# LiWentomng/OrientedRepPoints

Measured on AMD Instinct MI355X. Metric: images/sec (1024x1024 DOTA, R-50 FPN), higher is better.
Workload: dtype f32; 1 GPU; configs[1]: OrientedRepPoints R-50 FPN inference, 1024x1024 patch, 15 classes, bs=1/GPU, nms_pre=2000, score_thr=0.05, rnms iou_thr=0.4, max_per_img=2000; random-init weights, head biases calibrated to ~2000 dets/img; global_batch=1, parallelism=replicas x1 (image-parallel, no collective), images_in_flight_per_gpu=4

## Files before the change

include/orp_hip.h:

```cpp
#ifndef ORP_HIP_H_
#define ORP_HIP_H_

#include <stddef.h>
#include <stdint.h>

#ifdef __cplusplus
extern "C" {
#endif

#define ORP_OK 0
#define ORP_EINVAL (-1)
#define ORP_EWORKSPACE (-2)
#define ORP_ETOOBIG (-3)

const char* orp_version(void);

#define ORP_NMS_MAX_BOXES 131072
size_t orp_rnms_workspace_bytes(int n);
int orp_rnms(const float* dets, int n, float iou_thr, int flavor, int presorted, int order_out,
             int64_t* keep_out, int32_t* num_keep, void* workspace, size_t workspace_bytes, void* stream);

size_t orp_rnms_batched_workspace_bytes(int n_total, int nseg, int max_seg);
int orp_rnms_batched(const float* dets, int n_total, const int32_t* seg_offsets, int nseg, int max_seg,
                     float iou_thr, int flavor, int64_t* keep_out, int32_t* num_keep,
// ... 94 lines not shown
int orp_dcn_backward_multi(const orp_dcn_bwd_level* levels_host, int nlevels, int batch, int c_in, int c_out,
                           const float* weight, float* grad_weight, int need_input_grads, int kh, int kw, int stride_h,
                           int stride_w, int pad_h, int pad_w, int dil_h, int dil_w, void* workspace,
                           size_t workspace_bytes, void* stream);
int orp_dcn_backward_multi_ex(const orp_dcn_bwd_level* levels_host, const float* const* masks_host,
                              float* const* grad_masks_host, int io_dtype, int nlevels, int batch, int c_in, int c_out,
                              const float* weight, float* grad_weight, int need_input_grads, int kh, int kw, int stride_h,
                              int stride_w, int pad_h, int pad_w, int dil_h, int dil_w, void* workspace,
                              size_t workspace_bytes, void* stream);

int orp_dcn_im2col(const float* input, const float* offset, const float* mask, int batch, int c_in, int height,
                   int width, int kh, int kw, int stride_h, int stride_w, int pad_h, int pad_w, int dil_h, int dil_w,
                   int deformable_groups, float* columns, void* stream);
int orp_dcn_col2im(const float* grad_columns, const float* input, const float* offset, const float* mask, int batch,
                   int c_in, int height, int width, int kh, int kw, int stride_h, int stride_w, int pad_h, int pad_w,
                   int dil_h, int dil_w, int deformable_groups, float* grad_input, float* grad_offset, float* grad_mask,
                   void* stream);
int orp_dcn_im2col_f64(const double* input, const double* offset, const double* mask, int batch, int c_in, int height,
                       int width, int kh, int kw, int stride_h, int stride_w, int pad_h, int pad_w, int dil_h, int dil_w,
                       int deformable_groups, double* columns, void* stream);
int orp_dcn_col2im_f64(const double* grad_columns, const double* input, const double* offset, const double* mask, int batch,
                       int c_in, int height, int width, int kh, int kw, int stride_h, int stride_w, int pad_h, int pad_w,
                       int dil_h, int dil_w, int deformable_groups, double* grad_input, double* grad_offset, double* grad_mask,
                       void* stream);
int orp_dcn_col2im_nhwc(const float* grad_columns_t, const float* input_nhwc, const float* offset, int batch, int c_in,
                        int height, int width, int kh, int kw, int stride_h, int stride_w, int pad_h, int pad_w,
                        int dil_h, int dil_w, float* grad_input_nhwc, float* grad_offset, void* stream);

size_t orp_point_assign_workspace_bytes(int n);
int orp_point_assign(const float* points, int n, const float* gts, int k, float scale, int pos_num, int64_t* gt_inds,
                     void* workspace, size_t workspace_bytes, void* stream);
size_t orp_max_iou_assign_workspace_bytes(int k);
int orp_max_iou_assign(const float* overlaps_nk, int n, int k, float pos_iou_thr, float neg_iou_lo, float neg_iou_hi,
                       float min_pos_iou, int gt_max_assign_all, int64_t* gt_inds, float* max_overlaps,
                       void* workspace, size_t workspace_bytes, void* stream);
int orp_apaa_feature_dissimilarity(const float* const* feats_host, const int* heights_host, const int* widths_host,
                                   const float* strides_host, int num_levels, int channels, const float* pts18,
                                   const int32_t* img_index, const int32_t* level_index, int p, float* out,
                                   void* stream);
int orp_apaa_select(const float* quality, const int64_t* pos_gt_inds, const int32_t* pos_level, int p, int num_gt,
                    int num_level, int per_level_topk, double top_ratio, uint8_t* keep, void* stream);

typedef struct { const float* data; float* grad; int height; int width; float stride; } orp_level_desc;
int orp_pointset_target(const int64_t* gt_inds, const uint8_t* valid, int batch, int n, const float* gt_boxes,
                        const int64_t* gt_labels, const int32_t* gt_offset, const float* proposals, int dim,
                        float pos_weight, int64_t* labels, float* label_weights, float* rbbox_gt, float* pos_proposals,
                        float* proposal_weights, int64_t* gt_inds_out, int32_t* counts, void* stream);
int orp_points_from_offsets(const orp_level_desc* levels_host, int nlevels, int batch, int channels, int mode, float* out,
                            void* stream);
int orp_gather_levels(const orp_level_desc* levels_host, int nlevels, int batch, int channels, const int64_t* index, int p,
                      int mode, float* out, void* stream);
int orp_gather_levels_backward(const orp_level_desc* levels_host, int nlevels, int batch, int channels, const int64_t* index,
                               int p, int mode, const float* grad_out, void* stream);
int orp_outline_samples(const float* corners, int p, int n, const float* ratios, float* out, void* stream);

int orp_border_rows(const float* pts18, const float* gt8, const float* weight, int p, float* row_sum, float* row_cnt,
                    float* gdir, void* stream);
int orp_giou_rows(const float* gious, const float* grad18, const float* weight, const int64_t* seg, const float* denom, int p,
                  float loss_weight, float* contrib, float* gsave, void* stream);
int orp_segment_finish(const float* row_val, const float* row_cnt, const int64_t* seg, int p, int nseg, const float* denom,
                       float loss_weight, int mode, float* loss, float* scale, void* stream);

size_t orp_poly_nms_f64_workspace_bytes(int n);
int orp_poly_nms_f64(const double* dets_sorted, int n, double iou_thr, int64_t* keep_out, int32_t* num_keep,
                     void* workspace, size_t workspace_bytes, void* stream);

size_t orp_poly_nms_f64_batched_workspace_bytes(int n_total, int nseg, int max_seg);
int orp_poly_nms_f64_batched(const double* dets, int n_total, const int32_t* seg_offsets, int nseg, int max_seg,
                             double iou_thr, int hbb_prefilter, int presorted, int64_t* keep_out, int32_t* num_keep,
                             void* workspace, size_t workspace_bytes, void* stream);

int orp_scene_tiles(const uint8_t* scene, int height, int width, long long row_stride_bytes, const int32_t* origins,
                    int num_tiles, int tile, const float* mean_host, const float* std_host, int to_rgb, int out_dtype,
                    void* out, void* stream);
int orp_scene_tiles_resized(const uint8_t* scene, int height, int width, long long row_stride_bytes, const int32_t* origins,
                            int num_tiles, int src_w, int src_h, int new_w, int new_h, int pad_w, int pad_h, const int32_t* x_i0,
                            const float* x_w1, const int32_t* y_i0, const float* y_w1, const float* mean_host,
                            const float* std_host, int to_rgb, int out_dtype, void* out, void* stream);
int orp_scene_tiles_flip(const uint8_t* scene, int height, int width, long long row_stride_bytes, const int32_t* origins,
                         int num_tiles, int tile, const float* mean_host, const float* std_host, int to_rgb, int out_dtype,
                         void* out, void* stream);
int orp_scene_tiles_resized_flip(const uint8_t* scene, int height, int width, long long row_stride_bytes, const int32_t* origins,
                                 int num_tiles, int src_w, int src_h, int new_w, int new_h, int pad_w, int pad_h,
                                 const int32_t* x_i0, const float* x_w1, const int32_t* y_i0, const float* y_w1,
                                 const float* mean_host, const float* std_host, int to_rgb, int out_dtype, void* out,
                                 void* stream);
size_t orp_scene_collect_workspace_bytes(int num_tiles, int num_classes);
int orp_scene_collect(const float* packed, int num_tiles, int max_rows, const int32_t* origins, double rate, int num_classes,
                      int capacity_rows, double* dets, int32_t* seg_offsets, int32_t* src, int32_t* flag, void* workspace,
                      size_t workspace_bytes, void* stream);

int orp_voc_best_match_f64(const double* dets, const int32_t* det_image, int num_dets, const double* gts,
                           const int32_t* gt_offsets, int num_images, double* ovmax, int32_t* jmax, void* stream);

int orp_soft_rnms_host(const float* dets_host, int m, float iou_thr, int method, float sigma, float min_score,
                       float* out_host, int* num_out);

typedef struct { const float* input; float* output; int height; int width; } orp_norm_level;
size_t orp_groupnorm_workspace_bytes(const orp_norm_level* levels_host, int nlevels, int batch, int channels, int groups);
int orp_groupnorm_act_multi(const orp_norm_level* levels_host, int nlevels, int batch, int channels, int groups,
                            const float* gamma, const float* beta, float eps, int relu, void* workspace,
                            size_t workspace_bytes, void* stream);
int orp_groupnorm_act_multi_ex(const orp_norm_level* levels, const float* const* gammas_host,
                               const float* const* betas_host, int nlevels, int batch, int channels, int groups,
                               float eps, int relu, void* workspace, size_t workspace_bytes, void* stream);
int orp_groupnorm_act_multi_nhwc(const orp_norm_level* levels, const float* const* gammas_host,
                                 const float* const* betas_host, float* const* nhwc_out_host, int nlevels, int batch,
                                 int channels, int groups, float eps, int relu, void* workspace, size_t workspace_bytes,
                                 void* stream);
size_t orp_groupnorm_cl_workspace_bytes(const orp_norm_level* levels_host, int nlevels, int batch, int channels, int groups);
int orp_groupnorm_act_multi_cl(const orp_norm_level* levels, const float* const* gammas_host, const float* const* betas_host,
                               int nlevels, int batch, int channels, int groups, float eps, int relu, void* workspace,
                               size_t workspace_bytes, void* stream);
int orp_groupnorm_act_multi_cl_amax(const orp_norm_level* levels, const float* const* gammas_host, const float* const* betas_host,
                                    int nlevels, int batch, int channels, int groups, float eps, int relu, const int* slots_host,
                                    uint32_t* amax_out, int nslots, void* workspace, size_t workspace_bytes, void* stream);
int orp_groupnorm_act_multi_train(const orp_norm_level* levels, const float* const* gammas_host,
                                  const float* const* betas_host, int nlevels, int batch, int channels, int groups,
                                  float eps, int relu, float* stats, void* workspace, size_t workspace_bytes, void* stream);
size_t orp_groupnorm_backward_workspace_bytes(const orp_norm_level* levels_host, int nlevels, int batch, int channels, int groups);
int orp_groupnorm_act_multi_backward(const orp_norm_level* levels, const float* const* grad_outputs_host,
                                     float* const* grad_inputs_host, const float* const* gammas_host,
                                     const float* const* betas_host, float* const* dgammas_host, float* const* dbetas_host,
                                     int nlevels, int batch, int channels, int groups, int relu, const float* stats,
                                     void* workspace, size_t workspace_bytes, void* stream);
int orp_affine_act(const float* x, const float* residual, const float* scale, const float* shift, float* y, int batch,
                   int channels, int hw, int relu, void* stream);
int orp_affine2_act(const float* x, const float* residual, const float* scale, const float* shift, const float* scale2,
                    const float* shift2, float* y, int batch, int channels, int hw, int relu, void* stream);
int orp_affine_relu_maxpool(const float* x, const float* scale, const float* shift, float* y, int batch, int channels,
                            int height, int width, void* stream);
size_t orp_fpn_topdown_workspace_bytes(const orp_norm_level* levels, int nlevels, int batch, int channels, int groups);
int orp_fpn_topdown_nhwc(const orp_norm_level* levels, const float* const* gammas_host, const float* const* betas_host,
                         int nlevels, int batch, int channels, int groups, float eps, uint32_t* amax_out, void* workspace,
                         size_t workspace_bytes, void* stream);

typedef struct { const float* input; const float* residual; float* output; float* output2; int height; int width; } orp_bias_level;
int orp_bias_act_multi(const orp_bias_level* levels_host, int nlevels, int batch, int channels, const float* bias,
                       const float* sub, int relu, void* stream);

size_t orp_conv1x1_packed_floats(int c_in);
int orp_conv1x1_ok(int c_in, int c_out);
int orp_conv1x1_pack_weight(const float* weight, int c_out, int c_in, float* packed, void* stream);
int orp_conv1x1_multi(const orp_bias_level* levels_host, int nlevels, int batch, int c_in, int c_out,
                      const float* weight_packed, const float* bias, const float* sub, int relu, void* stream);

int orp_conv1x1_bn_act_ok(int c_in, int c_out);
int orp_conv1x1_bn_act_pays(int c_in, int c_out, int hw, int batch, int has_residual);
int orp_conv1x1_bn_act_tile(int c_in, int c_out, int hw, int batch, int* tile_channels, int* tile_positions);
int orp_conv1x1_bn_act(const float* x, const float* weight_t, const float* scale, const float* shift, const float* residual,
                       const float* scale2, const float* shift2, float* y, int batch, int c_in, int c_out, int hw, int relu,
                       void* stream);

int orp_conv3x3_small_ok(int c_in, int c_out);
int orp_conv3x3_small_multi(const orp_norm_level* levels_host, int nlevels, int batch, int c_in, int c_out,
                            const float* weight_packed, void* stream);
int orp_conv3x3_small_multi_ex(const orp_norm_level* levels_host, const float* const* weights_packed_host, int nlevels,
                               int batch, int c_in, int c_out, void* stream);
size_t orp_conv3x3_small_workspace_bytes(const orp_norm_level* levels_host, const int* strides_host, int nlevels, int batch,
                                         int c_out);
int orp_conv3x3_small_multi_strided(const orp_norm_level* levels_host, const float* const* weights_packed_host,
                                    const int* strides_host, int nlevels, int batch, int c_in, int c_out, void* workspace,
                                    size_t workspace_bytes, void* stream);

typedef struct { const float* input_a; const float* input_b; float* output_a; float* output_b; int height; int width; } orp_conv_level;
int orp_conv_split_ok(int c_in, int c_out, int kh, int kw);
int orp_conv_split_multi(const orp_conv_level* levels_host, int nlevels, int batch, int c_in, int c_out,
                         const float* weight_a_packed, const float* weight_b_packed, const float* bias_a, const float* bias_b,
                         int relu, int kh, int kw, int stride_h, int stride_w, int pad_h, int pad_w, int dil_h, int dil_w,
                         int out_layout, int nprod, void* workspace, size_t workspace_bytes, const uint32_t* amax_in,
                         int amax_stride, void* stream);
int orp_conv_split_multi_ex(const orp_conv_level* levels_host, const float* const* weights_packed_host,
                            const float* const* biases_host, int nlevels, int batch, int c_in, int c_out, int relu, int kh, int kw,
                            int stride_h, int stride_w, int pad_h, int pad_w, int dil_h, int dil_w, int out_layout, int nprod,
                            void* workspace, size_t workspace_bytes, const uint32_t* amax_in, void* stream);
size_t orp_conv_split_gn_partial_floats(const orp_conv_level* levels_host, int nlevels, int batch, int groups, int nlayers);
int orp_conv_split_multi_gn(const orp_conv_level* levels_host, int nlevels, int batch, int c_in, int c_out,
                            const float* weight_a_packed, const float* weight_b_packed, int kh, int kw, int pad_h, int pad_w,
                            int dil_h, int dil_w, int nprod, const float* coef_in, int relu_in, float* partials,
                            size_t partial_floats, int groups, void* workspace, size_t workspace_bytes, const uint32_t* amax_in,
                            int amax_stride, int amax_count, void* stream);
int orp_conv_split_gn_finish(const orp_conv_level* levels_host, int nlevels, int batch, int channels, int groups, int nlayers,
                             float eps, const float* const* gammas_host, const float* const* betas_host, const float* partials,
                             float* coef_out, uint32_t* bound_out, void* stream);
int orp_affine_act_multi_cl(const orp_norm_level* levels, int nlevels, int batch, int channels, const float* coef, int relu,
                            const uint32_t* bound_in, int nsets, int per_set, uint32_t* slot_out, void* stream);
int orp_conv_split_set_halo(int on);
int orp_conv_split_halo_tile(const orp_conv_level* levels_host, int nlevels, int batch, int c_in, int c_out, int kh, int kw, int stride,
                             int pad, int dil, int nprod, int* th, int* tw);
int orp_nchw_to_nhwc_multi(const orp_norm_level* levels_host, int nlevels, int batch, int channels, void* stream);
int orp_nchw_to_nhwc_multi_amax(const orp_norm_level* levels_host, int nlevels, int batch, int channels, const int* slots_host,
                                uint32_t* amax_out, int nslots, int reset, void* stream);

typedef struct { const float* input; const float* grad_output; int height; int width; } orp_wgrad_level;
int orp_conv_wgrad_split_ok(int c_in, int c_out, int kh, int kw);
size_t orp_conv_wgrad_split_workspace_bytes(const orp_wgrad_level* levels_host, int nlevels, int batch, int kh, int kw);
int orp_conv_wgrad_split(const orp_wgrad_level* levels_host, int nlevels, int batch, int c_in, int c_out, int kh, int kw,
                         int pad_h, int pad_w, int dil_h, int dil_w, const uint32_t* amax_x, const uint32_t* amax_g,
                         float* grad_weight, void* workspace, size_t workspace_bytes, void* stream);

typedef struct {
  const float* sig_all;
  const int64_t* cand;
  const float* boxes;
  const float* reppoints;
  int m0, n, flip, img_width;
  double scale;
} orp_pp_view;
size_t orp_pp_select_scratch_bytes(int n, int nms_pre, int nlevels);
int orp_pp_select(const float* sig_all, int num_classes, int n, const int* level_offsets_host, int nlevels, int nms_pre,
                  int64_t* cand, void* scratch, size_t scratch_bytes, void* stream);
int orp_pp_gather(const float* pts_all, const int64_t* cand, int m0, int n, const int* level_offsets_host,
                  const int* level_widths_host, const float* level_strides_host, int nlevels, float* pts_xy,
                  float* centers, float* strides, float* reppoints, void* stream);
size_t orp_pp_compact_scratch_bytes(int m0);
int orp_pp_compact(const float* sig_all, const int64_t* cand, int m0, int n, int num_classes, const float* boxes,
                   float score_thr, int capacity, float* dets, int32_t* sel_cand, int32_t* sel_label, int32_t* seg2,
                   int32_t* total, void* scratch, size_t scratch_bytes, void* stream);
size_t orp_pp_compact_views_scratch_bytes(int total_m0);
int orp_pp_compact_views(const orp_pp_view* views_host, int num_views, int num_classes, float score_thr, int capacity,
                         float* boxes_all, float* reppoints_all, float* dets, int32_t* sel_cand, int32_t* sel_label,
                         int32_t* seg2, int32_t* total, void* scratch, size_t scratch_bytes, void* stream);
int orp_pp_pack(const int64_t* keep, const int32_t* num_keep, const float* dets, const int32_t* sel_cand,
                const int32_t* sel_label, const float* boxes, const float* reppoints, const int32_t* total, int capacity,
                int max_out, float* packed, void* stream);

int orp_profile_enable(int on);
int orp_debug_amax_log(uint32_t* log, int capacity_launches);
int orp_profile_read(int slot, double* total_ms, int* count, int reset);

#ifdef __cplusplus
}
#endif
#endif
```

orientedreppoints_amd/_lib.py:

```python
import ctypes
import os

import torch

_HERE = os.path.dirname(os.path.abspath(__file__))
LIB_PATH = os.environ.get("ORP_HIP_LIB") or os.path.join(_HERE, "csrc", "liborp_hip.so")

ORP_OK, ORP_EINVAL, ORP_EWORKSPACE, ORP_ETOOBIG = 0, -1, -2, -3
ORP_NMS_MAX_BOXES = 131072

_vp = ctypes.c_void_p
_i = ctypes.c_int
_f = ctypes.c_float
_sz = ctypes.c_size_t

_SIGNATURES = {
    "orp_version": (ctypes.c_char_p, []),
    "orp_rnms_workspace_bytes": (_sz, [_i]),
    "orp_rnms": (_i, [_vp, _i, _f, _i, _i, _i, _vp, _vp, _vp, _sz, _vp]),
    "orp_rnms_batched_workspace_bytes": (_sz, [_i, _i, _i]),
    "orp_rnms_batched": (_i, [_vp, _i, _vp, _i, _i, _f, _i, _vp, _vp, _vp, _sz, _vp]),
    "_poly_nms": (None, [_vp, _vp, _vp, _i, _i, _f, _i]),
    "_overlaps": (None, [_vp, _vp, _vp, _i, _i, _i]),
    "orp_quad_iou_matrix": (_i, [_vp, _i, _vp, _i, _i, _i, _vp, _vp]),
    "orp_poly_overlaps": (_i, [_vp, _i, _vp, _i, _vp, _vp]),
    "orp_box_iou_rotated": (_i, [_vp, _i, _vp, _i, _vp, _vp]),
    "orp_box_iou_rotated_host": (_i, [_vp, _i, _vp, _i, _vp]),
    "orp_minarearect": (_i, [_vp, _i, _vp, _vp]),
    "orp_minarearect_decode": (_i, [_vp, _i, _vp, _vp, _vp, _vp]),
    "orp_libm_eval": (_i, [_vp, _vp, ctypes.c_long, _i, _vp, _vp]),
    "orp_convex_iou": (_i, [_vp, _i, _vp, _i, _vp, _vp]),
    "orp_convex_giou": (_i, [_vp, _vp, _i, _vp, _vp]),
    "orp_points_justify": (_i, [_vp, _i, _vp, _i, _vp, _vp]),
    "orp_points_in_quad_aligned": (_i, [_vp, _vp, _i, _vp, _vp]),
    "orp_chamfer2d_forward": (_i, [_vp, _vp, _i, _i, _i, _vp, _vp, _vp, _vp, _vp]),
    "orp_chamfer2d_backward": (_i, [_vp, _vp, _i, _i, _i, _vp, _vp, _vp, _vp, _vp, _vp, _vp]),
    "orp_sigmoid_focal_loss_forward": (_i, [_vp, _vp, _i, _i, _f, _f, _vp, _vp]),
    "orp_sigmoid_focal_loss_backward": (_i, [_vp, _vp, _vp, _i, _i, _f, _f, _vp, _vp]),
    "orp_sigmoid_focal_loss_forward_f64": (_i, [_vp, _vp, _i, _i, _f, _f, _vp, _vp]),
    "orp_sigmoid_focal_loss_backward_f64": (_i, [_vp, _vp, _vp, _i, _i, _f, _f, _vp, _vp]),
    "orp_point_assign_workspace_bytes": (_sz, [_i]),
    "orp_point_assign": (_i, [_vp, _i, _vp, _i, _f, _i, _vp, _vp, _sz, _vp]),
    "orp_max_iou_assign_workspace_bytes": (_sz, [_i]),
    "orp_max_iou_assign": (_i, [_vp, _i, _i, _f, _f, _f, _f, _i, _vp, _vp, _vp, _sz, _vp]),
    "orp_apaa_feature_dissimilarity": (_i, [_vp, _vp, _vp, _vp, _i, _i, _vp, _vp, _vp, _i, _vp, _vp]),
    "orp_apaa_select": (_i, [_vp, _vp, _vp, _i, _i, _i, _i, ctypes.c_double, _vp, _vp]),
    "orp_pointset_target": (_i, [_vp, _vp, _i, _i, _vp, _vp, _vp, _vp, _i, _f, _vp, _vp, _vp, _vp, _vp, _vp, _vp, _vp]),
    "orp_points_from_offsets": (_i, [_vp, _i, _i, _i, _i, _vp, _vp]),
    "orp_gather_levels": (_i, [_vp, _i, _i, _i, _vp, _i, _i, _vp, _vp]),
    "orp_gather_levels_backward": (_i, [_vp, _i, _i, _i, _vp, _i, _i, _vp, _vp]),
    "orp_outline_samples": (_i, [_vp, _i, _i, _vp, _vp, _vp]),
    "orp_profile_enable": (_i, [_i]),
    "orp_profile_read": (_i, [_i, _vp, _vp, _i]),
    "orp_dcn_fast_path_ok": (_i, [_i, _i, _i, _i, _i, _i]),
    "orp_dcn_pack_weight": (_i, [_vp, _i, _i, _i, _i, _vp, _vp]),
    "orp_dcn_packed_weight_floats": (_sz, [_i, _i, _i, _i]),
    "orp_dcn_set_split_mode": (_i, [_i]),
    "orp_dcn_get_split_mode": (_i, []),
    "orp_dcn_forward_workspace_bytes": (_sz, [_vp, _i, _i, _i, _i]),
    "orp_dcn_forward_multi": (_i, [_vp, _i, _i, _i, _i, _vp] + [_i] * 10 + [_vp, _sz, _vp]),
    "orp_dcn_forward_multi_ex": (_i, [_vp, _vp, _i, _i, _i, _i, _vp, _vp] + [_i] * 11 + [_vp, _sz, _vp]),
    "orp_dcn_forward_pair": (_i, [_vp, _vp, _vp, _i, _i, _i, _i, _vp, _vp, _vp, _vp] + [_i] * 11 + [_vp, _sz, _vp]),
    "orp_dcn_head_packed_floats": (_sz, []),
    "orp_dcn_pack_head_weight": (_i, [_vp, _i, _vp, _vp]),
    "orp_dcn_forward_pair_heads": (_i, [_vp, _vp, _i, _i, _vp, _vp, _vp] + [_i] * 9 + [_vp, _sz, _vp]),
    "orp_dcn_half_path_ok": (_i, [_i, _i, _i, _i, _i, _i]),
    "orp_dcn_pack_weight_h": (_i, [_vp, _i, _i, _i, _i, _vp, _i, _vp]),
    "orp_dcn_forward_h_tile_rows": (_i, [ctypes.c_long, _i]),
    "orp_dcn_forward_h_wave_specialised": (_i, []),
    "orp_dcn_forward_h_workspace_bytes": (_sz, [_vp, _i, _i, _i, _i]),
    "orp_dcn_forward_multi_h": (_i, [_vp, _vp, _i, _i, _i, _i, _vp, _vp] + [_i] * 12 + [_vp, _sz, _vp]),
    "orp_dcn_im2col": (_i, [_vp, _vp, _vp] + [_i] * 13 + [_vp, _vp]),
    "orp_dcn_col2im": (_i, [_vp, _vp, _vp, _vp] + [_i] * 13 + [_vp, _vp, _vp, _vp]),
    "orp_dcn_im2col_f64": (_i, [_vp, _vp, _vp] + [_i] * 13 + [_vp, _vp]),
    "orp_dcn_col2im_f64": (_i, [_vp, _vp, _vp, _vp] + [_i] * 13 + [_vp, _vp, _vp, _vp]),
    "orp_dcn_col2im_nhwc": (_i, [_vp, _vp, _vp] + [_i] * 12 + [_vp, _vp, _vp]),
    "orp_dcn_forward_direct": (_i, [_vp] * 6 + [_i] * 15 + [_vp]),
    "orp_dcn_backward_mfma_ok": (_i, [_i] * 6),
    "orp_dcn_backward_workspace_bytes": (_sz, [_vp] + [_i] * 10),
    "orp_dcn_backward_multi": (_i, [_vp, _i, _i, _i, _i, _vp, _vp] + [_i] * 9 + [_vp, _sz, _vp]),
    "orp_dcn_backward_multi_ex": (_i, [_vp, _vp, _vp, _i, _i, _i, _i, _i, _vp, _vp] + [_i] * 9 + [_vp, _sz, _vp]),
    "orp_poly_nms_f64_workspace_bytes": (_sz, [_i]),
    "orp_poly_nms_f64": (_i, [_vp, _i, ctypes.c_double, _vp, _vp, _vp, _sz, _vp]),
    "orp_poly_nms_f64_batched_workspace_bytes": (_sz, [_i, _i, _i]),
    "orp_poly_nms_f64_batched": (_i, [_vp, _i, _vp, _i, _i, ctypes.c_double, _i, _i, _vp, _vp, _vp, _sz, _vp]),
    "orp_scene_tiles": (_i, [_vp, _i, _i, ctypes.c_longlong, _vp, _i, _i, _vp, _vp, _i, _i, _vp, _vp]),
    "orp_scene_tiles_resized": (_i, [_vp, _i, _i, ctypes.c_longlong, _vp, _i, _i, _i, _i, _i, _i, _i, _vp, _vp, _vp, _vp, _vp, _vp, _i,
                                     _i, _vp, _vp]),
    "orp_scene_tiles_flip": (_i, [_vp, _i, _i, ctypes.c_longlong, _vp, _i, _i, _vp, _vp, _i, _i, _vp, _vp]),
    "orp_scene_tiles_resized_flip": (_i, [_vp, _i, _i, ctypes.c_longlong, _vp, _i, _i, _i, _i, _i, _i, _i, _vp, _vp, _vp, _vp, _vp,
                                          _vp, _i, _i, _vp, _vp]),
    "orp_scene_collect_workspace_bytes": (_sz, [_i, _i]),
    "orp_scene_collect": (_i, [_vp, _i, _i, _vp, ctypes.c_double, _i, _i, _vp, _vp, _vp, _vp, _vp, _sz, _vp]),
    "orp_soft_rnms_host": (_i, [_vp, _i, _f, _i, _f, _f, _vp, _vp]),
    "orp_conv1x1_packed_floats": (_sz, [_i]),
    "orp_conv1x1_ok": (_i, [_i, _i]),
    "orp_conv1x1_pack_weight": (_i, [_vp, _i, _i, _vp, _vp]),
    "orp_conv1x1_multi": (_i, [_vp, _i, _i, _i, _i, _vp, _vp, _vp, _i, _vp]),
    "orp_conv1x1_bn_act_ok": (_i, [_i, _i]),
    "orp_conv1x1_bn_act_pays": (_i, [_i, _i, _i, _i, _i]),
    "orp_conv1x1_bn_act_tile": (_i, [_i, _i, _i, _i, _vp, _vp]),
    "orp_conv1x1_bn_act": (_i, [_vp, _vp, _vp, _vp, _vp, _vp, _vp, _vp, _i, _i, _i, _i, _i, _vp]),
    "orp_pp_select_scratch_bytes": (_sz, [_i, _i, _i]),
    "orp_pp_select": (_i, [_vp, _i, _i, _vp, _i, _i, _vp, _vp, _sz, _vp]),
    "orp_pp_gather": (_i, [_vp, _vp, _i, _i, _vp, _vp, _vp, _i, _vp, _vp, _vp, _vp, _vp]),
    "orp_pp_compact_scratch_bytes": (_sz, [_i]),
    "orp_pp_compact": (_i, [_vp, _vp, _i, _i, _i, _vp, _f, _i, _vp, _vp, _vp, _vp, _vp, _vp, _sz, _vp]),
    "orp_pp_compact_views_scratch_bytes": (_sz, [_i]),
    "orp_pp_compact_views": (_i, [_vp, _i, _i, _f, _i, _vp, _vp, _vp, _vp, _vp, _vp, _vp, _vp, _sz, _vp]),
    "orp_pp_pack": (_i, [_vp, _vp, _vp, _vp, _vp, _vp, _vp, _vp, _i, _i, _vp, _vp]),
    "orp_groupnorm_workspace_bytes": (_sz, [_vp, _i, _i, _i, _i]),
    "orp_groupnorm_act_multi": (_i, [_vp, _i, _i, _i, _i, _vp, _vp, _f, _i, _vp, _sz, _vp]),
    "orp_groupnorm_act_multi_ex": (_i, [_vp, _vp, _vp, _i, _i, _i, _i, _f, _i, _vp, _sz, _vp]),
    "orp_groupnorm_act_multi_nhwc": (_i, [_vp, _vp, _vp, _vp, _i, _i, _i, _i, _f, _i, _vp, _sz, _vp]),
    "orp_groupnorm_act_multi_train": (_i, [_vp, _vp, _vp, _i, _i, _i, _i, _f, _i, _vp, _vp, _sz, _vp]),
    "orp_groupnorm_backward_workspace_bytes": (_sz, [_vp, _i, _i, _i, _i]),
    "orp_groupnorm_act_multi_backward": (_i, [_vp, _vp, _vp, _vp, _vp, _vp, _vp, _i, _i, _i, _i, _i, _vp, _vp, _sz, _vp]),
    "orp_voc_best_match_f64": (_i, [_vp, _vp, _i, _vp, _vp, _i, _vp, _vp, _vp]),
    "orp_affine_act": (_i, [_vp, _vp, _vp, _vp, _vp, _i, _i, _i, _i, _vp]),
    "orp_affine2_act": (_i, [_vp, _vp, _vp, _vp, _vp, _vp, _vp, _i, _i, _i, _i, _vp]),
    "orp_affine_relu_maxpool": (_i, [_vp, _vp, _vp, _vp, _i, _i, _i, _i, _vp]),
    "orp_fpn_topdown_workspace_bytes": (_sz, [_vp, _i, _i, _i, _i]),
    "orp_fpn_topdown_nhwc": (_i, [_vp, _vp, _vp, _i, _i, _i, _i, _f, _vp, _vp, _sz, _vp]),
    "orp_bias_act_multi": (_i, [_vp, _i, _i, _i, _vp, _vp, _i, _vp]),
    "orp_conv3x3_small_ok": (_i, [_i, _i]),
    "orp_conv3x3_small_multi": (_i, [_vp, _i, _i, _i, _i, _vp, _vp]),
    "orp_conv3x3_small_multi_ex": (_i, [_vp, _vp, _i, _i, _i, _i, _vp]),
    "orp_border_rows": (_i, [_vp, _vp, _vp, _i, _vp, _vp, _vp, _vp]),
    "orp_giou_rows": (_i, [_vp, _vp, _vp, _vp, _vp, _i, _f, _vp, _vp, _vp]),
    "orp_segment_finish": (_i, [_vp, _vp, _vp, _i, _i, _vp, _f, _i, _vp, _vp, _vp]),
    "orp_conv3x3_small_workspace_bytes": (ctypes.c_size_t, [_vp, _vp, _i, _i, _i]),
    "orp_conv3x3_small_multi_strided": (_i, [_vp, _vp, _vp, _i, _i, _i, _i, _vp, ctypes.c_size_t, _vp]),
    "orp_conv_split_ok": (_i, [_i, _i, _i, _i]),
    "orp_conv_split_multi": (_i, [_vp, _i, _i, _i, _i, _vp, _vp, _vp, _vp] + [_i] * 11 + [_vp, _sz, _vp, _i, _vp]),
    "orp_conv_split_multi_ex": (_i, [_vp, _vp, _vp, _i, _i, _i, _i] + [_i] * 11 + [_vp, _sz, _vp, _vp]),
    "orp_conv_split_set_halo": (_i, [_i]),
    "orp_conv_split_halo_tile": (_i, [_vp] + [_i] * 10 + [_vp, _vp]),
    "orp_conv_wgrad_split_ok": (_i, [_i, _i, _i, _i]),
    "orp_conv_wgrad_split_workspace_bytes": (_sz, [_vp, _i, _i, _i, _i]),
    "orp_conv_wgrad_split": (_i, [_vp, _i, _i, _i, _i, _i, _i, _i, _i, _i, _i, _vp, _vp, _vp, _vp, _sz, _vp]),
    "orp_nchw_to_nhwc_multi_amax": (_i, [_vp, _i, _i, _i, _vp, _vp, _i, _i, _vp]),
    "orp_groupnorm_act_multi_cl_amax": (_i, [_vp, _vp, _vp, _i, _i, _i, _i, _f, _i, _vp, _vp, _i, _vp, _sz, _vp]),
    "orp_dcn_forward_pair_amax": (_i, [_vp, _vp, _vp, _i, _i, _i, _i, _vp, _vp, _vp, _vp] + [_i] * 11 + [_vp, _sz, _vp, _i, _vp]),
    "orp_nchw_to_nhwc_multi": (_i, [_vp, _i, _i, _i, _vp]),
    "orp_groupnorm_cl_workspace_bytes": (_sz, [_vp, _i, _i, _i, _i]),
    "orp_groupnorm_act_multi_cl": (_i, [_vp, _vp, _vp, _i, _i, _i, _i, _f, _i, _vp, _sz, _vp]),
    "orp_debug_amax_log": (_i, [_vp, _i]),
    "orp_conv_split_gn_partial_floats": (_sz, [_vp, _i, _i, _i, _i]),
    "orp_conv_split_multi_gn": (_i, [_vp, _i, _i, _i, _i, _vp, _vp] + [_i] * 7 + [_vp, _i, _vp, _sz, _i, _vp, _sz, _vp, _i, _i, _vp]),
    "orp_conv_split_gn_finish": (_i, [_vp, _i, _i, _i, _i, _i, _f, _vp, _vp, _vp, _vp, _vp, _vp]),
    "orp_affine_act_multi_cl": (_i, [_vp, _i, _i, _i, _vp, _i, _vp, _i, _i, _vp, _vp]),
}

_lib = None


class OrpHipError(RuntimeError):
    pass


def lib():
    global _lib
    if _lib is None:
        if not os.path.exists(LIB_PATH):
            raise OrpHipError(
                "orientedreppoints_amd: HIP library %s is missing. Build it with "
                "`python -c 'import __graft_entry__ as g; g.build()'` (hipcc --offload-arch=gfx950). "
                "There is no CPU fallback for the hot path." % LIB_PATH)
        L = ctypes.CDLL(LIB_PATH)
        for name, (res, args) in _SIGNATURES.items():
            fn = getattr(L, name)
            fn.restype = res
            fn.argtypes = args
        _lib = L
    return _lib


def check(rc, what):
    if rc != ORP_OK:
        names = {ORP_EINVAL: "ORP_EINVAL", ORP_EWORKSPACE: "ORP_EWORKSPACE", ORP_ETOOBIG: "ORP_ETOOBIG"}
        raise OrpHipError("%s failed: %s" % (what, names.get(rc, "hipError %d" % rc)))


def ptr(t):
    if t is None:
        return None
    assert t.is_contiguous(), "orientedreppoints_amd: tensor must be contiguous"
    return ctypes.c_void_p(t.data_ptr())


def stream_of(t):
    return ctypes.c_void_p(torch.cuda.current_stream(t.device).cuda_stream)


def require_cuda(t, name):
    if not isinstance(t, torch.Tensor) or not t.is_cuda:
        raise TypeError("%s must be a CUDA tensor" % name)


_workspaces = {}
_keepalive = None


def workspace(device, nbytes):
    nbytes = max(int(nbytes), 1)
    if torch.cuda.is_current_stream_capturing():
        return torch.empty(nbytes, dtype=torch.uint8, device=device)
    idx = device.index if device.index is not None else torch.cuda.current_device()
    key = (idx, torch.cuda.current_stream(device).cuda_stream)
    w = _workspaces.get(key)
    if w is None or w.numel() < nbytes:
        if key not in _workspaces and len(_workspaces) >= 32:
            _workspaces.pop(next(iter(_workspaces)))
        w = torch.empty(max(nbytes, 1 << 20), dtype=torch.uint8, device=device)
        _workspaces[key] = w
    return w


def keep_for_graph(t):
    if _keepalive is not None and t is not None:
        _keepalive.append(t)
    return t
```

orientedreppoints_amd/build.py:

```python
import concurrent.futures
import os
import subprocess

HERE = os.path.dirname(os.path.abspath(__file__))
CSRC = os.path.join(HERE, "csrc")
LIB = os.path.join(CSRC, "liborp_hip.so")
HIPCC = os.environ.get("HIPCC", "/opt/rocm/bin/hipcc")
ARCH = "gfx950"

NO_PACKED_FP32 = ["-Xclang", "-target-feature", "-Xclang", "-packed-fp32-ops"]
COMMON = ["--offload-arch=" + ARCH, "-O3", "-std=c++17", "-fPIC", "-Wall", "-Wno-unused-function",
          "-Wno-unused-result", "-Wno-unused-value",
          "-Wno-bitwise-instead-of-logical"]
if os.environ.get("ORP_PACKED_FP32", "0") != "1":
    COMMON = COMMON + NO_PACKED_FP32
SOURCES = [
    ("orp_nms.hip", ["-ffp-contract=off"]),
    ("orp_overlaps.hip", ["-ffp-contract=off"]),
    ("orp_minarearect.hip", ["-ffp-contract=off"]),
    ("orp_box_iou_rotated.hip", ["-ffp-contract=off"]),
    ("orp_convex.hip", ["-ffp-contract=off"]),
    ("orp_convex_giou.hip", ["-ffp-contract=off"]),
    ("orp_pointwise.hip", ["-ffp-contract=off"]),
    ("orp_assign.hip", ["-ffp-contract=off"]),
    ("orp_postproc.hip", ["-ffp-contract=off"]),
    ("orp_soft_rnms.hip", ["-ffp-contract=off"]),
    ("orp_scene.hip", ["-ffp-contract=off"]),
    ("orp_eval.hip", ["-ffp-contract=off"]),
    ("orp_train.hip", ["-ffp-contract=off"]),
    ("orp_norm.hip", []),
    ("orp_conv_small.hip", []),
    ("orp_conv1x1.hip", []),
    ("orp_conv1x1_bn.hip", []),
    ("orp_dcn.hip", []),
    ("orp_dcn_split.hip", ["-ffp-contract=off"]),
    ("orp_conv_split.hip", []),
    ("orp_conv_wgrad.hip", []),
    ("orp_dcn_half.hip", []),
    ("orp_dcn_bwd.hip", []),
    ("orp_dcn_bwd_mfma.hip", []),
    ("orp_prof.hip", []),
]
HEADERS = ["orp_affine.hpp", "orp_geom.hpp", "orp_quadfast.hpp", "orp_tile.hpp", "orp_hull.hpp", "orp_libm.hpp", "orp_prof.hpp", "orp_launch.hpp", "orp_dcn_split.hpp", "orp_dcn_common.hpp", "orp_range.hpp", os.path.join("..", "..", "include", "orp_hip.h")]


def _stale(target, deps):
    if not os.path.exists(target):
        return True
    t = os.path.getmtime(target)
    return any(os.path.getmtime(d) > t for d in deps if os.path.exists(d))


VERSION_SOURCE = "orp_overlaps.hip"


def build_id():
    import hashlib
    h = hashlib.sha1()
    names = sorted([s for s, _ in SOURCES] + [x for x in HEADERS])
    for n in names:
        path = os.path.join(CSRC, n)
        if os.path.exists(path):
            h.update(n.encode())
            h.update(open(path, "rb").read())
    return h.hexdigest()[:12]


def _compile(src, extra):
    obj = os.path.join(CSRC, os.path.splitext(src)[0] + ".o")
    deps = [os.path.join(CSRC, src)] + [os.path.join(CSRC, h) for h in HEADERS] + [os.path.abspath(__file__)]
    if src == VERSION_SOURCE:
        deps += [os.path.join(CSRC, s) for s, _ in SOURCES]
        extra = extra + ['-DORP_BUILD_ID="%s"' % build_id()]
    if _stale(obj, deps):
        cmd = [HIPCC] + COMMON + extra + ["-c", os.path.join(CSRC, src), "-o", obj]
        r = subprocess.run(cmd, cwd=CSRC, stderr=subprocess.PIPE, universal_newlines=True)
        err = "\n".join(l for l in r.stderr.splitlines() if "'-packed-fp32-ops' is not a recognized feature" not in l)
        if err.strip():
            import sys
            sys.stderr.write(err + "\n")
        if r.returncode != 0:
            raise subprocess.CalledProcessError(r.returncode, cmd)
    return obj


def build_hip(force=False, verbose=False):
    if not os.path.exists(HIPCC):
        raise RuntimeError("hipcc not found at %s: cannot build liborp_hip.so" % HIPCC)
    present = [(s, f) for s, f in SOURCES if os.path.exists(os.path.join(CSRC, s))]
    if force:
        for s, _ in present:
            o = os.path.join(CSRC, os.path.splitext(s)[0] + ".o")
            if os.path.exists(o):
                os.remove(o)
    with concurrent.futures.ThreadPoolExecutor(max_workers=min(8, len(present))) as ex:
        objs = list(ex.map(lambda sf: _compile(*sf), present))
    if _stale(LIB, objs):
        cmd = [HIPCC, "--offload-arch=" + ARCH, "-shared", "-fPIC"] + objs + ["-o", LIB]
        if verbose:
            print(" ".join(cmd))
        subprocess.check_call(cmd, cwd=CSRC)
    return LIB


if __name__ == "__main__":
    print(build_hip(verbose=True))
```

orientedreppoints_amd/csrc/orp_conv1x1_bn.hip:

```cpp
#include <hip/hip_runtime.h>
#include <stdint.h>

#include "../../include/orp_hip.h"
#include "orp_affine.hpp"

namespace {

constexpr int kThreads = 256;
constexpr int BK = 32;

typedef float f32x16 __attribute__((ext_vector_type(16)));

struct Args {
  const float* x;
  const float* wt;
  const float* scale; const float* shift;
  const float* res;
  const float* scale2; const float* shift2;
  float* y;
  int cin, cout, hw, relu;
  int ntm, ntn;
};

template <int WM, int WN, bool VEC, int MODE>
__global__ void __launch_bounds__(kThreads, 2)
conv1x1_bn_act_kernel(const Args P) {
  constexpr int BM = 64 * WM, BN = 64 * WN;
  constexpr int WV = BK * BM / 4 / kThreads, XV = BK * BN / 4 / kThreads;
  __shared__ __align__(16) float lds[BK * (BM + BN) + 4 * BM];
  float* Ws = lds;
  float* Xs = lds + BK * BM;
  float* Cs = Xs + BK * BN;

  const int tid = threadIdx.x;
  const int bid = blockIdx.x;
  const int mt = bid % P.ntm, rest = bid / P.ntm;
  const int nt = rest % P.ntn, b = rest / P.ntn;
  const int m0 = mt * BM, p0 = nt * BN;
  const int hw = P.hw, cout = P.cout;
  const float* xb = P.x + (size_t)b * P.cin * hw;
  if (tid < BM) {
    const int ch = min(m0 + tid, cout - 1);
    Cs[tid] = P.scale[ch]; Cs[BM + tid] = P.shift[ch];
    if (MODE == 2) { Cs[2 * BM + tid] = P.scale2[ch]; Cs[3 * BM + tid] = P.shift2[ch]; }
  }

  float4 wr[WV], xr[XV];
  int wcol[WV], xcol[XV];
#pragma unroll
  for (int i = 0; i < WV; i++) wcol[i] = min(m0 + ((tid + i * kThreads) % (BM / 4)) * 4, cout - 4);
#pragma unroll
  for (int i = 0; i < XV; i++) xcol[i] = p0 + ((tid + i * kThreads) % (BN / 4)) * 4;

  auto fetch = [&](int k0) {
#pragma unroll
    for (int i = 0; i < WV; i++) {
      const int row = (tid + i * kThreads) / (BM / 4);
      wr[i] = *reinterpret_cast<const float4*>(P.wt + (size_t)(k0 + row) * cout + wcol[i]);
    }
#pragma unroll
    for (int i = 0; i < XV; i++) {
      const int row = (tid + i * kThreads) / (BN / 4);
      const float* src = xb + (size_t)(k0 + row) * hw;
      if (VEC) {
        xr[i] = *reinterpret_cast<const float4*>(src + min(xcol[i], hw - 4));
      } else {
        xr[i].x = src[min(xcol[i], hw - 1)]; xr[i].y = src[min(xcol[i] + 1, hw - 1)];
        xr[i].z = src[min(xcol[i] + 2, hw - 1)]; xr[i].w = src[min(xcol[i] + 3, hw - 1)];
      }
    }
  };
  auto stage = [&]() {
#pragma unroll
    for (int i = 0; i < WV; i++) {
      const int idx = tid + i * kThreads;
      float4 v = wr[i];
      if (m0 + (idx % (BM / 4)) * 4 >= cout) v = make_float4(0.f, 0.f, 0.f, 0.f);
      *reinterpret_cast<float4*>(Ws + (idx / (BM / 4)) * BM + (idx % (BM / 4)) * 4) = v;
    }
#pragma unroll
    for (int i = 0; i < XV; i++) {
      const int idx = tid + i * kThreads;
      float4 v = xr[i];
      const int p = xcol[i];
      if (p >= hw) v.x = 0.f;
      if (p + 1 >= hw) v.y = 0.f;
      if (p + 2 >= hw) v.z = 0.f;
      if (p + 3 >= hw) v.w = 0.f;
      *reinterpret_cast<float4*>(Xs + (idx / (BN / 4)) * BN + (idx % (BN / 4)) * 4) = v;
    }
  };

  const int lane = tid & 63, wave = tid >> 6;
  const int half = lane >> 5, l31 = lane & 31;
  const int wm0 = (wave >> 1) * 32 * WM, wn0 = (wave & 1) * 32 * WN;
  f32x16 acc[WM][WN];
#pragma unroll
  for (int mi = 0; mi < WM; mi++)
#pragma unroll
    for (int ni = 0; ni < WN; ni++)
#pragma unroll
      for (int r = 0; r < 16; r++) acc[mi][ni][r] = 0.f;

  auto mma = [&]() {
    const float* wa = Ws + half * BM + wm0 + l31;
    const float* xa = Xs + half * BN + wn0 + l31;
#pragma unroll
    for (int kk = 0; kk < BK / 2; kk++) {
      float a[WM], bb[WN];
#pragma unroll
      for (int mi = 0; mi < WM; mi++) a[mi] = wa[kk * 2 * BM + mi * 32];
#pragma unroll
      for (int ni = 0; ni < WN; ni++) bb[ni] = xa[kk * 2 * BN + ni * 32];
#pragma unroll
      for (int mi = 0; mi < WM; mi++)
#pragma unroll
        for (int ni = 0; ni < WN; ni++) acc[mi][ni] = __builtin_amdgcn_mfma_f32_32x32x2f32(a[mi], bb[ni], acc[mi][ni], 0, 0, 0);
    }
  };

  const int nk = P.cin / BK;
  fetch(0);
  stage();
  __syncthreads();
  for (int t = 0; t + 1 < nk; t++) {
    fetch((t + 1) * BK);
    __builtin_amdgcn_sched_barrier(0);
    mma();
    __builtin_amdgcn_sched_barrier(0);
    __syncthreads();
    stage();
    __syncthreads();
  }

  const size_t plane0 = (size_t)b * cout;
  float rv[WM][WN][16];
  if (MODE) {
#pragma unroll
    for (int mi = 0; mi < WM; mi++)
#pragma unroll
      for (int ni = 0; ni < WN; ni++) {
        const int p = min(p0 + wn0 + 32 * ni + l31, hw - 1);
#pragma unroll
        for (int r = 0; r < 16; r++) {
          const int ch = min(m0 + wm0 + 32 * mi + 8 * (r >> 2) + 4 * half + (r & 3), cout - 1);
          rv[mi][ni][r] = P.res[(plane0 + ch) * hw + p];
        }
      }
  }
  __builtin_amdgcn_sched_barrier(0);
  mma();

#pragma unroll
  for (int mi = 0; mi < WM; mi++) {
#pragma unroll
    for (int g = 0; g < 4; g++) {
      const int chg = m0 + wm0 + 32 * mi + 8 * g + 4 * half;
      const float* cs = Cs + wm0 + 32 * mi + 8 * g + 4 * half;
      const float4 a4 = *reinterpret_cast<const float4*>(cs);
      const float4 b4 = *reinterpret_cast<const float4*>(cs + BM);
      const float av[4] = {a4.x, a4.y, a4.z, a4.w}, bv[4] = {b4.x, b4.y, b4.z, b4.w};
      float a2v[4] = {0.f, 0.f, 0.f, 0.f}, b2v[4] = {0.f, 0.f, 0.f, 0.f};
      if (MODE == 2) {
        const float4 c4 = *reinterpret_cast<const float4*>(cs + 2 * BM);
        const float4 d4 = *reinterpret_cast<const float4*>(cs + 3 * BM);
        a2v[0] = c4.x; a2v[1] = c4.y; a2v[2] = c4.z; a2v[3] = c4.w;
        b2v[0] = d4.x; b2v[1] = d4.y; b2v[2] = d4.z; b2v[3] = d4.w;
      }
#pragma unroll
      for (int ni = 0; ni < WN; ni++) {
        const int p = p0 + wn0 + 32 * ni + l31;
#pragma unroll
        for (int q = 0; q < 4; q++) {
          const int r = 4 * g + q;
          const float v = acc[mi][ni][r];
          float t;
          if (MODE == 0) t = affine_act(v, av[q], bv[q], P.relu);
          else if (MODE == 1) t = affine_res_act(v, av[q], bv[q], rv[mi][ni][r], P.relu);
          else t = affine_res_act(v, av[q], bv[q], affine_act(rv[mi][ni][r], a2v[q], b2v[q], 0), P.relu);
          if (chg < cout && p < hw) P.y[(plane0 + chg + q) * hw + p] = t;
        }
      }
    }
  }
}

struct Tile { int bm, bn; };

Tile pick_tile(int cout, int hw, int batch) {
  const Tile cand[3] = {{128, 128}, {64, 128}, {64, 64}};
  for (int i = 0; i < 3; i++) {
    const Tile t = cand[i];
    if (t.bm > ((cout + 63) / 64) * 64) continue;
    const long wgs = (long)((cout + t.bm - 1) / t.bm) * ((hw + t.bn - 1) / t.bn) * batch;
    if (wgs >= 512) return t;
  }
  return cand[2];
}

template <int WM, int WN, int MODE>
void launch_mode(const Args& A, int batch, bool vec, hipStream_t st) {
  const dim3 grid((unsigned)((long)A.ntm * A.ntn * batch));
  if (vec) hipLaunchKernelGGL((conv1x1_bn_act_kernel<WM, WN, true, MODE>), grid, dim3(kThreads), 0, st, A);
  else hipLaunchKernelGGL((conv1x1_bn_act_kernel<WM, WN, false, MODE>), grid, dim3(kThreads), 0, st, A);
}
template <int WM, int WN>
void launch(const Args& A, int batch, bool vec, hipStream_t st) {
  if (!A.res) launch_mode<WM, WN, 0>(A, batch, vec, st);
  else if (!A.scale2) launch_mode<WM, WN, 1>(A, batch, vec, st);
  else launch_mode<WM, WN, 2>(A, batch, vec, st);
}

}

extern "C" {

int orp_conv1x1_bn_act_ok(int c_in, int c_out) {
  return (c_in >= 64 && c_in <= 2048 && c_in % 32 == 0 && c_out >= 64 && c_out <= 4096 && c_out % 32 == 0) ? 1 : 0;
}

int orp_conv1x1_bn_act_tile(int c_in, int c_out, int hw, int batch, int* tile_channels, int* tile_positions) {
  if (!orp_conv1x1_bn_act_ok(c_in, c_out) || hw <= 0 || batch <= 0) return 0;
  const Tile t = pick_tile(c_out, hw, batch);
  if (tile_channels) *tile_channels = t.bm;
  if (tile_positions) *tile_positions = t.bn;
  return 1;
}

int orp_conv1x1_bn_act_pays(int c_in, int c_out, int hw, int batch, int has_residual) {
  if (!orp_conv1x1_bn_act_ok(c_in, c_out) || hw <= 0 || batch <= 0) return 0;
  (void)has_residual;
  static const struct { int cin, cout, hw_min, hw_max, batch; } paid[] = {
      {64, 64, 65536, 147456, 1},   {64, 64, 65536, 65536, 2},
      {256, 64, 65536, 147456, 1},  {256, 64, 65536, 65536, 2},
      {64, 256, 65536, 147456, 1},  {64, 256, 65536, 65536, 2},
      {256, 128, 65536, 147456, 1}, {256, 128, 65536, 65536, 2},
      {512, 128, 16384, 36864, 1},
      {128, 512, 16384, 36864, 1},  {128, 512, 16384, 16384, 2},
      {1024, 256, 4096, 4096, 1},
      {256, 1024, 4096, 9216, 1},   {256, 1024, 4096, 4096, 2},
      {512, 2048, 1024, 1024, 1},
  };
  for (const auto& s : paid)
    if (s.cin == c_in && s.cout == c_out && s.batch == batch && hw >= s.hw_min && hw <= s.hw_max) return 1;
  return 0;
}

int orp_conv1x1_bn_act(const float* x, const float* weight_t, const float* scale, const float* shift, const float* residual,
                       const float* scale2, const float* shift2, float* y, int batch, int c_in, int c_out, int hw, int relu,
                       void* stream) {
  if (!x || !weight_t || !scale || !shift || !y || batch <= 0 || hw <= 0 || !orp_conv1x1_bn_act_ok(c_in, c_out)) return ORP_EINVAL;
  if ((scale2 != nullptr) != (shift2 != nullptr) || (scale2 && !residual) || (const float*)y == x || (const float*)y == residual)
    return ORP_EINVAL;
  if ((uintptr_t)weight_t & 15) return ORP_EINVAL;
  const Tile t = pick_tile(c_out, hw, batch);
  Args A;
  A.x = x; A.wt = weight_t; A.scale = scale; A.shift = shift; A.res = residual; A.scale2 = scale2; A.shift2 = shift2; A.y = y;
  A.cin = c_in; A.cout = c_out; A.hw = hw; A.relu = relu ? 1 : 0;
  A.ntm = (c_out + t.bm - 1) / t.bm; A.ntn = (hw + t.bn - 1) / t.bn;
  if ((long)A.ntm * A.ntn * batch >= (1L << 31)) return ORP_ETOOBIG;
  const bool vec = (hw & 3) == 0 && ((uintptr_t)x & 15) == 0;
  hipStream_t st = (hipStream_t)stream;
  if (t.bm == 128) launch<2, 2>(A, batch, vec, st);
  else if (t.bn == 128) launch<1, 2>(A, batch, vec, st);
  else launch<1, 1>(A, batch, vec, st);
  hipError_t e = hipGetLastError();
  return e == hipSuccess ? ORP_OK : (int)e;
}

}
```

orientedreppoints_amd/csrc/orp_dcn_split.hip:

```cpp
#include <hip/hip_runtime.h>
#include <stdint.h>
#include <stdlib.h>

#include "orp_dcn_split.hpp"
#include "orp_range.hpp"
#include "orp_launch.hpp"
#include "orp_dcn_common.hpp"

namespace orp_split {
namespace {

typedef float floatx16 __attribute__((ext_vector_type(16)));
typedef __bf16 bf8 __attribute__((ext_vector_type(8)));
typedef _Float16 h8 __attribute__((ext_vector_type(8)));
typedef _Float16 h2 __attribute__((ext_vector_type(2)));

constexpr int kTapsMax = 9;
constexpr int CBS = 64;
constexpr int ASTRS = CBS + 8;
constexpr int NCH = CBS / 16;
constexpr int kThreadsS = 512;
constexpr int kInterleave = 4;

struct LevelK {
// ... 585 lines not shown
      const bool in = pix[i] >= 0;
      const float s[4] = {in ? x.x : 0.f, in ? x.y : 0.f, in ? x.z : 0.f, in ? x.w : 0.f};
      _Float16 hh[4], ll[4];
#pragma unroll
      for (int e = 0; e < 4; e++) {
        const float sv = s[e] * sx;
        hh[e] = (_Float16)sv;
        ll[e] = (_Float16)(sv - (float)hh[e]);
      }
      const h2 h01 = {hh[0], hh[1]}, h23 = {hh[2], hh[3]}, l01 = {ll[0], ll[1]}, l23 = {ll[2], ll[3]};
      uint16_t* dst = sA + (size_t)h * astr + k * CBS + c4;
      *reinterpret_cast<uint2*>(dst) = make_uint2(__builtin_bit_cast(unsigned, h01), __builtin_bit_cast(unsigned, h23));
      *reinterpret_cast<uint2*>(dst + plane) = make_uint2(__builtin_bit_cast(unsigned, l01), __builtin_bit_cast(unsigned, l23));
    }
  };

  const int n_wave = blockIdx.y * 256 + wave * 32;
  const int mrow = lane & 31, kg = lane >> 5;
  const bool live = n_wave < P.Cout;
  const uint16_t* wp = (L.planes ? L.planes : conv ? P.planes[1] : P.planes[0]) + ((size_t)kg * P.Cout + (live ? n_wave : 0) + mrow) * 8;
  const size_t wblk = (size_t)2 * P.Cout * 8;
  auto load_b = [&](int tap, int cb, int j, bf8 (&b)[3]) {
    const uint16_t* a = wp + ((size_t)tap * (P.Cin / 16) + cb * NCH + j) * wblk;
#pragma unroll
    for (int pl = 0; pl < 2; pl++) b[pl] = *reinterpret_cast<const bf8*>(a + (size_t)pl * P.plane_stride);
  };
  const uint16_t* abase[MT];
#pragma unroll
  for (int mt = 0; mt < MT; mt++) abase[mt] = sA + (size_t)(R.ty(mt * 32 + mrow) * hw + R.tx(mt * 32 + mrow)) * astr + 8 * kg;
  auto a_off = [&](int tap, int cb) { const int ki = tap / 3; return ((ki * hw + tap - 3 * ki) * astr + cb * CBS); };
  auto load_a = [&](int off, int j, bf8 (&a)[MT][3]) {
#pragma unroll
    for (int mt = 0; mt < MT; mt++)
#pragma unroll
      for (int pl = 0; pl < 2; pl++) a[mt][pl] = *reinterpret_cast<const bf8*>(abase[mt] + pl * plane + off + j * 16);
  };

  bf8 bq[NCH][3];
#pragma unroll
  for (int j = 0; j < NCH; j++) load_b(0, 0, j, bq[j]);
  __builtin_amdgcn_sched_barrier(0);
  float4 sv[kHaloStage];
  stage_issue(0, sv);
  __syncthreads();
  stage_store(0, sv);
  __syncthreads();

  floatx16 acc[MT], side[MT];
#pragma unroll
  for (int mt = 0; mt < MT; mt++) { acc[mt] = floatx16{0}; side[mt] = floatx16{0}; }
  const int ncb = P.Cin / CBS, nphase = 9 * ncb;
  int tap = 0, cb = 0, tap_n = 0, cb_n = 0;
  auto step = [&](int& t, int& c, int ph) {
    if (ph + 1 < nphase) { if (++c == ncb) { c = 0; t++; } }
  };
  step(tap_n, cb_n, 0);
  bf8 a[2][MT][3];
  load_a(a_off(0, 0), 0, a[0]);
  auto phase_body = [&]() __attribute__((always_inline)) {
    const int off = a_off(tap, cb), off_n = a_off(tap_n, cb_n);
#pragma unroll
    for (int j = 0; j < NCH; j++) {
      if (j + 1 < NCH) load_a(off, j + 1, a[(j + 1) & 1]);
      else             load_a(off_n, 0, a[0]);
      __builtin_amdgcn_sched_barrier(0);
      Products<0, 3, MT, OUT_NCHW, true, true>::run(acc, side, a[j & 1], bq[j]);
      __builtin_amdgcn_sched_barrier(0);
      load_b(tap_n, cb_n, j, bq[j]);
      __builtin_amdgcn_sched_barrier(0);
    }
  };
  int phase = 0;
#pragma unroll 1
  for (; phase + 1 < ncb; phase++) {
    stage_issue(phase + 1, sv);
    __builtin_amdgcn_sched_barrier(0);
    phase_body();
    stage_store(phase + 1, sv);
    __syncthreads();
    load_a(a_off(tap_n, cb_n), 0, a[0]);
    tap = tap_n; cb = cb_n;
    step(tap_n, cb_n, phase + 1);
  }
#pragma unroll 1
  for (; phase < nphase; phase++) {
    phase_body();
    tap = tap_n; cb = cb_n;
    step(tap_n, cb_n, phase + 1);
  }

  if (!live) return;
#pragma unroll
  for (int mt = 0; mt < MT; mt++) acc[mt] += side[mt];
  split_epilogue<MT, OUT_NCHW, true, !OUT_NCHW>(P, L, acc, R, conv, tile, total_tiles, n_wave, lane, kxw);
}

constexpr int kCoefCinMax = 512;
template <int MT, int NPL>
constexpr size_t split_smem() {
  return (size_t)2 * NPL * 32 * MT * ASTRS * 2 + (sizeof(float4) + sizeof(int4)) * 32 * MT * kTapsMax + sizeof(float) * 2 * kCoefCinMax;
}

template <int MT, int NPROD, bool OUT_NCHW, bool PLAIN>
hipError_t launch_one(const FwdS& P, int tiles, int nblk_n, hipStream_t st) {
  constexpr size_t smem = split_smem<MT, NPROD == 3 ? 2 : 3>();
  struct Tag {};
  hipError_t e = orp::set_max_dynamic_lds_once<Tag>(reinterpret_cast<const void*>(&dcn_fwd_split_kernel<MT, NPROD, OUT_NCHW, PLAIN>), smem);
  if (e != hipSuccess) return e;
  const int nx = P.nconv == 2 ? 4 : 8;
  const int per = (tiles + nx - 1) / nx;
  hipLaunchKernelGGL((dcn_fwd_split_kernel<MT, NPROD, OUT_NCHW, PLAIN>), dim3(per * 8, nblk_n), dim3(kThreadsS), smem, st, P, tiles);
  return hipGetLastError();
}

template <bool OUT_NCHW>
hipError_t launch_halo(const FwdS& P, int tiles, int nblk_n, hipStream_t st) {
  struct Tag {};
  hipError_t e = orp::set_max_dynamic_lds_once<Tag>(reinterpret_cast<const void*>(&conv_halo_kernel<OUT_NCHW>), halo_smem(kHaloCinMax));
  if (e != hipSuccess) return e;
  const int nx = P.nconv == 2 ? 4 : 8;
  const int per = (tiles + nx - 1) / nx;
  hipLaunchKernelGGL((conv_halo_kernel<OUT_NCHW>), dim3(per * 8, nblk_n), dim3(kThreadsS), halo_smem(P.Cin), st, P, tiles);
  return hipGetLastError();
}

template <int MT, int NPROD, bool PLAIN>
hipError_t launch_l(const FwdS& P, int tiles, int nblk_n, bool nchw, hipStream_t st) {
  return nchw ? launch_one<MT, NPROD, true, PLAIN>(P, tiles, nblk_n, st) : launch_one<MT, NPROD, false, PLAIN>(P, tiles, nblk_n, st);
}
template <int NPROD, bool PLAIN>
hipError_t launch_m(int MT, const FwdS& P, int tiles, int nblk_n, bool nchw, hipStream_t st) {
  return MT == 1 ? launch_l<1, NPROD, PLAIN>(P, tiles, nblk_n, nchw, st)
       : MT == 2 ? launch_l<2, NPROD, PLAIN>(P, tiles, nblk_n, nchw, st) : launch_l<3, NPROD, PLAIN>(P, tiles, nblk_n, nchw, st);
}

}

bool shape_ok(int c_in, int c_out, int kh, int kw) {
  return kh * kw <= kTapsMax && c_in % CBS == 0 && c_in >= CBS && c_out % 64 == 0 && c_out >= 64;
}

size_t plane_elems(int c_out, int c_in, int taps) { return (size_t)5 * c_out * c_in * taps + 8; }

const uint16_t* planes_of(const float* packed, int c_out, int c_in, int taps, int nprod) {
  const size_t n = (size_t)c_out * c_in * taps;
  const uint16_t* base = reinterpret_cast<const uint16_t*>(packed + 2 * n);
  return nprod == 3 ? base + 3 * n : base;
}
const float* wscale_of(const float* packed, int c_out, int c_in, int taps) {
  const size_t n = (size_t)c_out * c_in * taps;
  return reinterpret_cast<const float*>(reinterpret_cast<const uint16_t*>(packed + 2 * n) + 5 * n);
}

hipError_t pack_planes(const float* weight, int c_out, int c_in, int taps, uint16_t* planes, hipStream_t st) {
  const long total = (long)c_out * c_in * taps;
  int blocks = (int)((total + 255) / 256); if (blocks > 4096) blocks = 4096;
  hipLaunchKernelGGL(pack_planes_kernel, dim3(blocks), dim3(256), 0, st, weight, c_out, c_in, taps, planes);
  float* tail = reinterpret_cast<float*>(planes + 5 * total);
  unsigned* amax = reinterpret_cast<unsigned*>(tail + 1);
  hipError_t e = orp::fill_async(amax, 0, sizeof(unsigned), st);
  if (e != hipSuccess) return e;
  AbsMaxArgs M;
  long nb = (total / 4 + 256 * 8 - 1) / (256 * 8); if (nb < 1) nb = 1; if (nb > 512) nb = 512;
  for (int i = 0; i < kAbsMaxT; i++) { M.x[i] = weight; M.n[i] = i == 0 ? (size_t)total : 0; M.slot[i] = 0; M.bx0[i] = i == 0 ? 0 : (int)nb; }
  M.bx0[kAbsMaxT] = (int)nb; M.count = 1;
  hipLaunchKernelGGL(absmax_kernel, dim3((int)nb), dim3(256), 0, st, M, amax);
  hipLaunchKernelGGL(pack_planes16_kernel, dim3(blocks), dim3(256), 0, st, weight, c_out, c_in, taps, amax, planes + 3 * total, tail);
  return hipGetLastError();
}

static int g_halo = -1;
int halo_switch() {
  if (g_halo < 0) {
    const char* e = getenv("ORP_CONV_HALO");
    g_halo = (e && atoi(e) == 0) ? 0 : 1;
  }
  return g_halo;
}
void set_halo(int on) { g_halo = on < 0 ? -1 : on ? 1 : 0; }

bool halo_tiles(const Args& a, int on, int* th, int* tw) {
  bool plain = true;
  for (int i = 0; i < a.nlev; i++) plain = plain && !a.lv[i].off && !a.lv[i].mask;
  if (!on || !plain || a.nprod != 3 || a.kh != 3 || a.kw != 3 || a.sh != 1 || a.sw != 1 || a.dh != 1 || a.dw != 1 || a.ph != 1 || a.pw != 1 ||
      a.Cin % CBS != 0 || a.Cin > kHaloCinMax)
    return false;
  for (int i = 0; i < a.nlev; i++) { tw[i] = a.lv[i].W >= 16 ? 16 : 8; th[i] = 96 / tw[i]; }
  return true;
}

Plan plan(const Args& a) {
  Plan pl;
  pl.halo = halo_tiles(a, halo_switch(), pl.th, pl.tw) ? 1 : 0;
  if (pl.halo) {
    int tiles = 0;
    for (int i = 0; i < kMaxLevels; i++) { pl.tile0[i] = 0x7fffffff; pl.tpi[i] = 0; }
    for (int i = 0; i < a.nlev; i++) {
      pl.tile0[i] = tiles;
      pl.tpi[i] = ((a.lv[i].Ho + pl.th[i] - 1) / pl.th[i]) * ((a.lv[i].Wo + pl.tw[i] - 1) / pl.tw[i]);
      tiles += a.B * pl.tpi[i];
    }
    pl.MT = 3; pl.tiles = tiles;
    return pl;
  }
  long npos_all = 0;
  for (int i = 0; i < a.nlev; i++) npos_all += (long)a.B * a.lv[i].Ho * a.lv[i].Wo;
  const int cus = a.nconv == 2 ? 128 : 256;
  int MT = 1;
  long best = -1;
  for (int mt = 1; mt <= 3; mt++) {
    const long t = (npos_all + 32 * mt - 1) / (32 * mt) + a.nlev * (a.per_image ? a.B : 1);
    const long cost = ((t + cus - 1) / cus) * mt * (mt == 1 ? 130 : mt == 2 ? 110 : 100);
    if (best < 0 || cost < best) { best = cost; MT = mt; }
  }
  static const int force_mt = getenv("ORP_DCNS_MT") ? atoi(getenv("ORP_DCNS_MT")) : 0;
  if (force_mt >= 1 && force_mt <= 3) MT = force_mt;
  int tiles = 0;
  for (int i = 0; i < kMaxLevels; i++) { pl.tile0[i] = 0x7fffffff; pl.tpi[i] = 0; }
  for (int i = 0; i < a.nlev; i++) {
    const long hw = (long)a.lv[i].Ho * a.lv[i].Wo;
    pl.tile0[i] = tiles;
    if (a.per_image) {
      pl.tpi[i] = (int)((hw + 32 * MT - 1) / (32 * MT));
      tiles += a.B * pl.tpi[i];
    } else {
      tiles += (int)((a.B * hw + 32 * MT - 1) / (32 * MT));
    }
  }
  pl.MT = MT; pl.tiles = tiles;
  return pl;
}

static unsigned* g_amax_log = nullptr;
static int g_amax_log_cap = 0, g_amax_log_next = 0;
int set_amax_log(unsigned* log, int capacity_launches) {
  const int used = g_amax_log_next;
  g_amax_log = log; g_amax_log_cap = log ? capacity_launches : 0; g_amax_log_next = 0;
  return used;
}

hipError_t launch(const Args& a, hipStream_t st) {
  FwdS P;
  P.dbg = nullptr;
  if (a.nprod == 3 && g_amax_log && g_amax_log_next < g_amax_log_cap) P.dbg = g_amax_log + 4 * (g_amax_log_next++);
  P.nlev = a.nlev; P.B = a.B; P.Cin = a.Cin; P.Cout = a.Cout;
  P.kh = a.kh; P.kw = a.kw; P.sh = a.sh; P.sw = a.sw; P.ph = a.ph; P.pw = a.pw; P.dh = a.dh; P.dw = a.dw;
  P.planes[0] = a.planes[0]; P.planes[1] = a.planes[1]; P.bias[0] = a.bias[0]; P.bias[1] = a.bias[1];
  P.relu = a.relu; P.nconv = a.nconv;
  P.plane_stride = (size_t)a.Cout * a.Cin * a.kh * a.kw;
  P.coef_in = reinterpret_cast<const float2*>(a.coef_in); P.relu_in = a.relu_in;
  P.gn_part = reinterpret_cast<float4*>(a.gn_part); P.G = a.groups > 0 ? a.groups : 1;
  P.amax_count = a.amax_count > 1 ? a.amax_count : 1;
  if ((a.coef_in || a.gn_part) && (!a.per_image || a.lv[0].off != nullptr)) return hipErrorInvalidValue;
  if (a.coef_in && (a.Cin > kCoefCinMax || (a.nprod == 3 && !a.amax_in))) return hipErrorInvalidValue;
  if (a.gn_part && (a.out_nchw || a.groups <= 0 || a.Cout % a.groups != 0 || (32 % (a.Cout / a.groups)) != 0 || a.Cout / a.groups < 1 ||
                    a.relu || a.bias[0] || a.bias[1]))
    return hipErrorInvalidValue;
  const Plan pl = plan(a);
  const int MT = pl.MT, tiles = pl.tiles;
  for (int i = 0; i < a.nlev; i++) {
    LevelK& D = P.lv[i];
    D.x[0] = a.lv[i].x[0]; D.x[1] = a.lv[i].x[1]; D.off = a.lv[i].off; D.mask = a.lv[i].mask;
    D.out[0] = a.lv[i].out[0]; D.out[1] = a.lv[i].out[1];
    D.H = a.lv[i].H; D.W = a.lv[i].W; D.Ho = a.lv[i].Ho; D.Wo = a.lv[i].Wo;
    D.planes = a.nconv == 1 ? a.lv[i].planes : nullptr; D.bias = a.lv[i].bias; D.wscale = a.lv[i].wscale;
    D.tile0 = pl.tile0[i]; D.tpi = pl.tpi[i];
    D.th = pl.halo ? pl.th[i] : 0; D.tw = pl.halo ? pl.tw[i] : 0;
  }
  pad_level_slots(P.lv, a.nlev);
  const int nblk_n = (a.Cout + 255) / 256;
  bool plain = a.lv[0].off == nullptr;
  for (int i = 0; i < a.nlev; i++)
    if ((a.lv[i].off == nullptr) != plain || (plain && a.lv[i].mask)) return hipErrorInvalidValue;
  if (a.nprod == 3) {
    if ((!a.scratch && !a.amax_in) || !a.wscale[0] || (a.nconv == 2 && !a.wscale[1])) return hipErrorInvalidValue;
    for (int i = 0; i < a.nlev; i++) if (a.lv[i].mask) return hipErrorInvalidValue;
    if (a.amax_in) {
      P.amax = a.amax_in; P.amax_stride = a.amax_stride;
    } else {
      P.amax_count = 1;
      AbsMaxArgs M;
      int bx = 0, cnt = 0;
      for (int cv = 0; cv < a.nconv; cv++)
        for (int i = 0; i < a.nlev; i++) {
          M.x[cnt] = a.lv[i].x[cv]; M.n[cnt] = (size_t)a.B * a.lv[i].H * a.lv[i].W * a.Cin; M.slot[cnt] = cv; M.bx0[cnt] = bx;
          long nb = (long)((M.n[cnt] / 4 + 256 * 8 - 1) / (256 * 8)); if (nb < 1) nb = 1; if (nb > 512) nb = 512;
          bx += (int)nb; cnt++;
        }
      for (int i = cnt; i <= kAbsMaxT; i++) M.bx0[i] = bx;
      for (int i = cnt; i < kAbsMaxT; i++) { M.x[i] = M.x[0]; M.n[i] = 0; M.slot[i] = 0; }
      M.count = cnt;
      hipError_t e = orp::fill_async(a.scratch, 0, sizeof(unsigned) * (size_t)(2), st);
      if (e != hipSuccess) return e;
      hipLaunchKernelGGL(absmax_kernel, dim3(bx), dim3(256), 0, st, M, a.scratch);
      P.amax = a.scratch; P.amax_stride = 1;
    }
    P.wscale[0] = a.wscale[0]; P.wscale[1] = a.nconv == 2 ? a.wscale[1] : a.wscale[0];
    if (pl.halo) return a.out_nchw ? launch_halo<true>(P, tiles, nblk_n, st) : launch_halo<false>(P, tiles, nblk_n, st);
    return plain ? launch_m<3, true>(MT, P, tiles, nblk_n, a.out_nchw != 0, st)
                 : launch_m<3, false>(MT, P, tiles, nblk_n, a.out_nchw != 0, st);
  }
  P.amax = nullptr; P.amax_stride = 0; P.wscale[0] = P.wscale[1] = nullptr;
  if (plain)
    return a.nprod == 9 ? launch_m<9, true>(MT, P, tiles, nblk_n, a.out_nchw != 0, st)
                        : launch_m<6, true>(MT, P, tiles, nblk_n, a.out_nchw != 0, st);
  return a.nprod == 9 ? launch_m<9, false>(MT, P, tiles, nblk_n, a.out_nchw != 0, st)
                      : launch_m<6, false>(MT, P, tiles, nblk_n, a.out_nchw != 0, st);
}

}
```

orientedreppoints_amd/csrc/orp_dcn_split.hpp:

```cpp
#pragma once
#include <hip/hip_runtime.h>
#include <stddef.h>
#include <stdint.h>

namespace orp_split {

constexpr int kMaxLevels = 8;

struct Level {
  const float* x[2];
  const float* off;
  const float* mask;
  float* out[2];
  int H, W, Ho, Wo;
  const uint16_t* planes;
  const float* bias;
  const float* wscale;
};

struct Args {
  Level lv[kMaxLevels];
  int nlev, B, Cin, Cout;
  int kh, kw, sh, sw, ph, pw, dh, dw;
  const uint16_t* planes[2];
  const float* bias[2];
  int relu, nconv, out_nchw;
  int nprod;
  const float* wscale[2];
  unsigned* scratch;
  const unsigned* amax_in;
  int amax_stride;
  int amax_count = 0;
  int per_image = 0;
  const float* coef_in = nullptr;
  int relu_in = 0;
  float* gn_part = nullptr;
  int groups = 0;
};

struct Plan {
  int MT, tiles; int tile0[kMaxLevels], tpi[kMaxLevels];
  int halo;
  int th[kMaxLevels], tw[kMaxLevels];
};
Plan plan(const Args& a);
bool halo_tiles(const Args& a, int on, int* th, int* tw);
int halo_switch();
void set_halo(int on);

bool shape_ok(int c_in, int c_out, int kh, int kw);
size_t plane_elems(int c_out, int c_in, int taps);
const uint16_t* planes_of(const float* packed, int c_out, int c_in, int taps, int nprod);
const float* wscale_of(const float* packed, int c_out, int c_in, int taps);
hipError_t pack_planes(const float* weight , int c_out, int c_in, int taps, uint16_t* planes, hipStream_t st);
hipError_t launch(const Args& a, hipStream_t st);
int set_amax_log(unsigned* log, int capacity_launches);

}
```

orientedreppoints_amd/csrc/orp_norm.hip:

```cpp
#include <hip/hip_runtime.h>
#include <stdint.h>
#include <stdlib.h>

#include "../../include/orp_hip.h"
#include "orp_affine.hpp"
#include "orp_launch.hpp"
#include "orp_range.hpp"

namespace {

constexpr int kThreads = 256;
constexpr int kChunk = 4096;
constexpr int kMaxLevels = 8;
constexpr int kGnMaxLevels = 16;

struct GnLevel {
  const float* x; float* y;
  const float* gamma; const float* beta;
  int hw;
  int cpg;
  int chunk0;
};
struct GnParams {
  GnLevel lv[kGnMaxLevels];
// ... 164 lines not shown
  float* out[kGnMaxLevels];
  float* nchw[kGnMaxLevels];
  int bx0[kGnMaxLevels + 1];
};
__global__ void __launch_bounds__(kThreads)
gn_apply_nhwc_kernel(const GnParams P, const GnNhwc T) {
  __shared__ float tile[32][33];
  __shared__ float2 sStat[32];
  const int lvl = level_of([&](int i) { return T.bx0[i]; }, P.nlev, (int)blockIdx.x);
  const GnLevel& L = P.lv[lvl];
  const int hw = L.hw, cg = P.C / P.G;
  const int b = blockIdx.z, c0 = blockIdx.y * 32, p0 = ((int)blockIdx.x - T.bx0[lvl]) * 32;
  const int tx = threadIdx.x & 31, ty = threadIdx.x >> 5;
  const int ngrp = (32 + cg - 1) / cg;
  const int span = cg * hw;
  __shared__ float red[4];
  for (int gi = 0; gi < ngrp; gi++) {
    const int grp = c0 / cg + gi;
    if (grp >= P.G) break;
    const float2 mv = merge_span(P.partial + L.chunk0 + (size_t)(b * P.G + grp) * L.cpg, L.cpg, kChunk, span, 1, red);
    if (threadIdx.x == 0) sStat[gi] = make_float2(mv.x, rsqrtf(mv.y + P.eps));
  }
  __syncthreads();
  const float* src = L.x + (size_t)b * P.C * hw;
  float* nchw = T.nchw[lvl] ? T.nchw[lvl] + (size_t)b * P.C * hw : nullptr;
  for (int r = ty; r < 32; r += 8) {
    const int c = c0 + r, p = p0 + tx;
    float t = 0.f;
    if (c < P.C && p < hw) {
      const float2 st = sStat[r / cg];
      const float2 k = gn_coef(st.x, st.y, L.gamma[c], L.beta[c]);
      t = affine_act(src[(size_t)c * hw + p], k.x, k.y, P.relu);
      if (nchw) nchw[(size_t)c * hw + p] = t;
    }
    tile[r][tx] = t;
  }
  __syncthreads();
  float* dst = T.out[lvl] + (size_t)b * hw * P.C;
  for (int r = ty; r < 32; r += 8) {
    const int p = p0 + r, c = c0 + tx;
    if (p < hw && c < P.C) dst[(size_t)p * P.C + c] = tile[tx][r];
  }
}

constexpr int kTdMaxLevels = 4;
constexpr int kTdTiles = 8;
struct TdLevels {
  float* out[kTdMaxLevels];
  int width[kTdMaxLevels];
  int bx0[kTdMaxLevels + 1];
  float2* stats;
  unsigned* amax;
};

__global__ void __launch_bounds__(kThreads)
gn_merge_kernel(const GnParams P, const TdLevels T) {
  __shared__ float red[4];
  const int bg = blockIdx.x, lvl = blockIdx.y;
  const GnLevel& L = P.lv[lvl];
  const int span = (P.C / P.G) * L.hw;
  if (bg == 0 && lvl == 0 && threadIdx.x == 0 && T.amax) *T.amax = 0u;
  const float2 mv = merge_span(P.partial + L.chunk0 + (size_t)bg * L.cpg, L.cpg, kChunk, span, 1, red);
  if (threadIdx.x == 0) T.stats[(size_t)lvl * P.B * P.G + bg] = make_float2(mv.x, rsqrtf(mv.y + P.eps));
}

template <int NL>
__device__ __forceinline__ unsigned td_tiles(const GnParams& P, const TdLevels& T, int lvl, int b, int c0, int bx, float (*tile)[33],
                                             const float2 (*sStat)[32]) {
  const int cg = P.C / P.G;
  const int tx = threadIdx.x & 31, ty = threadIdx.x >> 5;
  const int hw = P.lv[lvl].hw;
  float ca[NL][4], cb[NL][4];
  const float* src[NL];
#pragma unroll
  for (int sh = 0; sh < NL; sh++) {
    const GnLevel& L = P.lv[lvl + sh];
    src[sh] = L.x + ((size_t)b * P.C + c0 + ty) * L.hw;
#pragma unroll
    for (int i = 0; i < 4; i++) {
      const int r = ty + 8 * i, c = c0 + r;
      const float2 st = sStat[sh][r / cg];
      const float2 k = gn_coef(st.x, st.y, L.gamma[c], L.beta[c]);
      ca[sh][i] = k.x; cb[sh][i] = k.y;
    }
  }
  float* dst = T.out[lvl] + (size_t)b * hw * P.C;
  unsigned m = 0u;
#pragma unroll 1
  for (int it = 0; it < kTdTiles; it++) {
    const int p0 = (bx * kTdTiles + it) * 32;
    if (p0 >= hw) break;
    const int p = min(p0 + tx, hw - 1);
    const int h = p / T.width[lvl], w = p - h * T.width[lvl];
    float x[NL][4];
#pragma unroll
    for (int sh = 0; sh < NL; sh++) {
      const size_t hwj = (size_t)P.lv[lvl + sh].hw;
      const float* q = src[sh] + (size_t)(h >> sh) * T.width[lvl + sh] + (w >> sh);
#pragma unroll
      for (int i = 0; i < 4; i++) x[sh][i] = q[(size_t)(8 * i) * hwj];
    }
#pragma unroll
    for (int i = 0; i < 4; i++) {
      float t = affine_act(x[NL - 1][i], ca[NL - 1][i], cb[NL - 1][i], 0);
#pragma unroll
      for (int sh = NL - 2; sh >= 0; sh--) {
        float g = affine_act(x[sh][i], ca[sh][i], cb[sh][i], 0);
        g += t;
        t = g;
      }
      if (p0 + tx >= hw) t = 0.f;
      tile[ty + 8 * i][tx] = t;
      m = max(m, orp::range_bits(t));
    }
    __syncthreads();
#pragma unroll
    for (int r = ty; r < 32; r += 8) {
      const int pp = p0 + r, c = c0 + tx;
      if (pp < hw) dst[(size_t)pp * P.C + c] = tile[tx][r];
    }
    __syncthreads();
  }
  return m;
}

__global__ void __launch_bounds__(kThreads)
fpn_topdown_nhwc_kernel(const GnParams P, const TdLevels T) {
  __shared__ float tile[32][33];
  __shared__ float2 sStat[kTdMaxLevels][32];
  const int lvl = level_of([&](int i) { return T.bx0[i]; }, P.nlev, (int)blockIdx.x);
  const int cg = P.C / P.G;
  const int b = blockIdx.z, c0 = blockIdx.y * 32, bx = (int)blockIdx.x - T.bx0[lvl];
  const int ngrp = 32 / cg;
  const int nl = P.nlev - lvl;
  if ((int)threadIdx.x < nl * ngrp) {
    const int sh = threadIdx.x / ngrp, gi = threadIdx.x - sh * ngrp;
    sStat[sh][gi] = T.stats[(size_t)(lvl + sh) * P.B * P.G + b * P.G + c0 / cg + gi];
  }
  __syncthreads();
  unsigned m;
  switch (nl) {
    case 1: m = td_tiles<1>(P, T, lvl, b, c0, bx, tile, sStat); break;
    case 2: m = td_tiles<2>(P, T, lvl, b, c0, bx, tile, sStat); break;
    case 3: m = td_tiles<3>(P, T, lvl, b, c0, bx, tile, sStat); break;
    default: m = td_tiles<4>(P, T, lvl, b, c0, bx, tile, sStat); break;
  }
  if (T.amax) {
    __shared__ unsigned redm[4];
    const unsigned mx = block_max(m, redm);
    if (threadIdx.x == 0) orp::range_raise(T.amax, mx);
  }
}

__global__ void __launch_bounds__(kThreads)
affine_act_kernel(const float* __restrict__ x, const float* __restrict__ res, const float* __restrict__ scale,
                  const float* __restrict__ shift, float* __restrict__ y, int C, int hw, int relu) {
  const int plane = blockIdx.y;
  const int c = plane % C;
  const float a = scale[c], b = shift[c];
  const size_t base = (size_t)plane * hw;
  if ((hw & 3) == 0) {
    const int hw4 = hw >> 2;
    const float4* x4 = reinterpret_cast<const float4*>(x + base);
    const float4* r4 = res ? reinterpret_cast<const float4*>(res + base) : nullptr;
    float4* y4 = reinterpret_cast<float4*>(y + base);
    for (int i = blockIdx.x * blockDim.x + threadIdx.x; i < hw4; i += gridDim.x * blockDim.x) {
      float4 t = x4[i];
      affine_act4(t, a, b, 0);
      if (r4) { const float4 r = r4[i]; t.x += r.x; t.y += r.y; t.z += r.z; t.w += r.w; }
      if (relu) relu4(t);
      y4[i] = t;
    }
  } else {
    for (int i = blockIdx.x * blockDim.x + threadIdx.x; i < hw; i += gridDim.x * blockDim.x) {
      y[base + i] = res ? affine_res_act(x[base + i], a, b, res[base + i], relu) : affine_act(x[base + i], a, b, relu);
    }
  }
}

__global__ void __launch_bounds__(kThreads)
affine2_act_kernel(const float* __restrict__ x, const float* __restrict__ res, const float* __restrict__ scale,
                   const float* __restrict__ shift, const float* __restrict__ scale2, const float* __restrict__ shift2,
                   float* __restrict__ y, int C, int hw, int relu) {
  const int plane = blockIdx.y;
  const int c = plane % C;
  const float a = scale[c], b = shift[c];
  const float a2 = scale2[c], b2 = shift2[c];
  const size_t base = (size_t)plane * hw;
  if ((hw & 3) == 0) {
    const int hw4 = hw >> 2;
    const float4* x4 = reinterpret_cast<const float4*>(x + base);
    const float4* r4 = reinterpret_cast<const float4*>(res + base);
    float4* y4 = reinterpret_cast<float4*>(y + base);
    for (int i = blockIdx.x * blockDim.x + threadIdx.x; i < hw4; i += gridDim.x * blockDim.x) {
      float4 t = x4[i];
      float4 r = r4[i];
      affine_act4(t, a, b, 0);
      affine_act4(r, a2, b2, 0);
      t.x += r.x; t.y += r.y; t.z += r.z; t.w += r.w;
      if (relu) relu4(t);
      y4[i] = t;
    }
  } else {
    for (int i = blockIdx.x * blockDim.x + threadIdx.x; i < hw; i += gridDim.x * blockDim.x) {
      y[base + i] = affine_res_act(x[base + i], a, b, affine_act(res[base + i], a2, b2, 0), relu);
    }
  }
}

constexpr int kPoolRows = 4;
template <bool kVec>
__global__ void __launch_bounds__(kThreads)
affine_relu_maxpool_kernel(const float* __restrict__ x, const float* __restrict__ scale, const float* __restrict__ shift,
                           float* __restrict__ y, int C, int H, int W, int Ho, int Wo, int nq, int nitems) {
  const int plane = blockIdx.y;
  const int c = plane % C;
  const float a = scale[c], b = shift[c];
  const float* src = x + (size_t)plane * H * W;
  float* dst = y + (size_t)plane * Ho * Wo;
  for (int it = blockIdx.x * blockDim.x + threadIdx.x; it < nitems; it += gridDim.x * blockDim.x) {
    const int s = it / nq, q = it - s * nq;
    const int col = 4 * q;
    const int ho0 = s * kPoolRows;
    auto load_row = [&](int row, float (&v)[5]) {
      if (row < 0 || row >= H) { v[0] = v[1] = v[2] = v[3] = v[4] = 0.f; return; }
      const float* p = src + (size_t)row * W + col;
      float t0, t1, t2, t3, t4;
      if (kVec) {
        const float4 f = *reinterpret_cast<const float4*>(p);
        t1 = f.x; t2 = f.y; t3 = f.z; t4 = f.w;
      } else {
        t1 = p[0];
        t2 = (col + 1 < W) ? p[1] : 0.f; t3 = (col + 2 < W) ? p[2] : 0.f; t4 = (col + 3 < W) ? p[3] : 0.f;
      }
      t0 = (col > 0) ? p[-1] : 0.f;
      v[0] = fmaxf(t0 * a + b, 0.f); v[1] = fmaxf(t1 * a + b, 0.f); v[2] = fmaxf(t2 * a + b, 0.f);
      v[3] = fmaxf(t3 * a + b, 0.f); v[4] = fmaxf(t4 * a + b, 0.f);
      if (col == 0) v[0] = 0.f;
      if (!kVec) { if (col + 1 >= W) v[2] = 0.f; if (col + 2 >= W) v[3] = 0.f; if (col + 3 >= W) v[4] = 0.f; }
    };
    float top[5];
    load_row(2 * ho0 - 1, top);
#pragma unroll
    for (int k = 0; k < kPoolRows; k++) {
      const int ho = ho0 + k;
      if (ho < Ho) {
        float mid[5], bot[5];
        load_row(2 * ho, mid);
        load_row(2 * ho + 1, bot);
        float m[5];
#pragma unroll
        for (int u = 0; u < 5; u++) { m[u] = fmaxf(fmaxf(top[u], mid[u]), bot[u]); top[u] = bot[u]; }
        const float o0 = fmaxf(fmaxf(m[0], m[1]), m[2]), o1 = fmaxf(fmaxf(m[2], m[3]), m[4]);
        float* d = dst + (size_t)ho * Wo + 2 * q;
        if (kVec) {
          *reinterpret_cast<float2*>(d) = make_float2(o0, o1);
        } else {
          d[0] = o0;
          if (2 * q + 1 < Wo) d[1] = o1;
        }
      }
    }
  }
}

struct BiasLevel {
  const float* x; const float* res; float* y; float* y2;
  int hw;
  int bx0;
};
struct BiasParams {
  BiasLevel lv[kMaxLevels];
  int nlev, C, relu;
  const float* bias; const float* sub;
};
__global__ void __launch_bounds__(kThreads)
bias_act_multi_kernel(const BiasParams P) {
  int l = 0;
#pragma unroll
  for (int i = 1; i < kMaxLevels; i++) l = (i < P.nlev && (int)blockIdx.x >= P.lv[i].bx0) ? i : l;
  const BiasLevel L = P.lv[l];
  const int plane = blockIdx.y;
  const int c = plane % P.C;
  const float b = P.bias ? P.bias[c] : 0.f;
  const float sb = P.sub ? P.sub[c] : 0.f;
  const size_t base = (size_t)plane * L.hw;
  const int bx = blockIdx.x - L.bx0;
  const int nbx = ((l + 1 < P.nlev) ? P.lv[l + 1].bx0 : (int)gridDim.x) - L.bx0;
  if ((L.hw & 3) == 0) {
    const int hw4 = L.hw >> 2;
    const float4* x4 = reinterpret_cast<const float4*>(L.x + base);
    const float4* r4 = L.res ? reinterpret_cast<const float4*>(L.res + base) : nullptr;
    float4* y4 = reinterpret_cast<float4*>(L.y + base);
    float4* z4 = L.y2 ? reinterpret_cast<float4*>(L.y2 + base) : nullptr;
    for (int i = bx * kThreads + threadIdx.x; i < hw4; i += nbx * kThreads) {
      float4 t = x4[i];
      t.x += b; t.y += b; t.z += b; t.w += b;
      if (r4) { const float4 r = r4[i]; t.x += r.x; t.y += r.y; t.z += r.z; t.w += r.w; }
      if (P.relu) relu4(t);
      y4[i] = t;
      if (z4) { t.x -= sb; t.y -= sb; t.z -= sb; t.w -= sb; z4[i] = t; }
    }
  } else {
    for (int i = bx * kThreads + threadIdx.x; i < L.hw; i += nbx * kThreads) {
      float t = L.x[base + i] + b;
      if (L.res) t += L.res[base + i];
      if (P.relu) t = fmaxf(t, 0.f);
      L.y[base + i] = t;
      if (L.y2) L.y2[base + i] = t - sb;
    }
  }
}

__global__ void __launch_bounds__(kThreads)
gn_bwd_partial_kernel(const GnParams P) {
  __shared__ float red[4];
  const ChunkGeom g = locate(P, blockIdx.x);
  const GnLevel& L = P.lv[g.lvl];
  const int cg = P.C / P.G;
  const float2 st = P.stats[(size_t)g.lvl * P.B * P.G + g.bg];
  const float mean = st.x, rstd = st.y;
  const float* x = L.x + (size_t)g.bg * g.span + g.n0;
  const float* y = L.y + (size_t)g.bg * g.span + g.n0;
  const float* dy = P.dy[g.lvl] + (size_t)g.bg * g.span + g.n0;
  const int c_first = g.n0 / L.hw, c_last = (g.n0 + g.n - 1) / L.hw;
  for (int cl = c_first; cl <= c_last; cl++) {
    const int e0 = max(cl * L.hw - g.n0, 0), e1 = min((cl + 1) * L.hw - g.n0, g.n);
    float s1 = 0.f, s2 = 0.f;
    for (int e = e0 + threadIdx.x; e < e1; e += kThreads) {
// ... 335 lines not shown
  if (channels % 32 != 0 || 32 % (channels / groups) != 0 || batch > 65535) return ORP_EINVAL;
  if (!workspace || workspace_bytes < sizeof(float2) * (size_t)chunks) return ORP_EWORKSPACE;
  GnNhwc T;
  int bx = 0;
  if (!set_affine(P, gammas_host, betas_host, nlevels)) return ORP_EINVAL;
  for (int i = 0; i < nlevels; i++) {
    if (!nhwc_out_host[i]) return ORP_EINVAL;
    T.out[i] = nhwc_out_host[i];
    T.nchw[i] = levels[i].output;
    T.bx0[i] = bx;
    bx += (P.lv[i].hw + 31) / 32;
  }
  for (int i = nlevels; i <= kGnMaxLevels; i++) T.bx0[i] = 0x7fffffff;
  for (int i = nlevels; i < kGnMaxLevels; i++) { T.out[i] = T.out[0]; T.nchw[i] = nullptr; }
  P.eps = eps; P.relu = relu;
  P.partial = reinterpret_cast<float2*>(workspace);
  P.stats = nullptr;
  hipStream_t st = (hipStream_t)stream;
  hipLaunchKernelGGL(gn_stats_kernel, dim3(chunks), dim3(kThreads), 0, st, P);
  hipLaunchKernelGGL(gn_apply_nhwc_kernel, dim3(bx, channels / 32, batch), dim3(kThreads), 0, st, P, T);
  return launch_status();
}

static size_t gn_cl_stat_offset(size_t chunks, int groups) { return (sizeof(float2) * chunks * groups + 255) & ~(size_t)255; }

size_t orp_groupnorm_cl_workspace_bytes(const orp_norm_level* levels, int nlevels, int batch, int channels, int groups) {
  GnClParams P;
  const int chunks = fill_cl(levels, nlevels, batch, channels, groups, P);
  if (chunks <= 0) return 0;
  return ((gn_cl_stat_offset(chunks, groups) + sizeof(float2) * (size_t)nlevels * batch * groups + 255) & ~(size_t)255) +
         sizeof(float) * (size_t)chunks * groups;
}

static int gn_cl_impl(const orp_norm_level* levels, const float* const* gammas_host, const float* const* betas_host,
                      int nlevels, int batch, int channels, int groups, float eps, int relu, const int* slots_host,
                      uint32_t* amax_out, int nslots, void* workspace, size_t workspace_bytes, void* stream) {
  GnClParams P;
  const int chunks = fill_cl(levels, nlevels, batch, channels, groups, P);
  if (const int rc = fill_status(chunks)) return rc;
  if (!gammas_host || !betas_host) return ORP_EINVAL;
  if (amax_out && (!slots_host || nslots <= 0)) return ORP_EINVAL;
  const size_t stat_off = gn_cl_stat_offset(chunks, groups);
  const size_t pmax_off = (stat_off + sizeof(float2) * (size_t)nlevels * batch * groups + 255) & ~(size_t)255;
  const size_t need = amax_out ? pmax_off + sizeof(float) * (size_t)chunks * groups : pmax_off;
  if (!workspace || workspace_bytes < need) return ORP_EWORKSPACE;
  if (!set_affine(P, gammas_host, betas_host, nlevels)) return ORP_EINVAL;
  for (int i = 0; i < nlevels; i++) {
    if (amax_out && (slots_host[i] < 0 || slots_host[i] >= nslots)) return ORP_EINVAL;
    P.slot[i] = amax_out ? slots_host[i] : 0;
  }
  for (int i = nlevels; i < kGnMaxLevels; i++) P.slot[i] = 0;
  P.eps = eps; P.relu = relu;
  P.partial = reinterpret_cast<float2*>(workspace);
  P.stats = reinterpret_cast<float2*>(reinterpret_cast<char*>(workspace) + stat_off);
  P.pmax = amax_out ? reinterpret_cast<float*>(reinterpret_cast<char*>(workspace) + pmax_off) : nullptr;
  P.amax = amax_out;
  hipStream_t st = (hipStream_t)stream;
  if (amax_out) {
    const hipError_t me = orp::fill_async(amax_out, 0, sizeof(unsigned) * (size_t)(nslots), st);
    if (me != hipSuccess) return (int)me;
  }
  hipLaunchKernelGGL(gn_cl_stats_kernel, dim3(chunks), dim3(kThreads), 0, st, P);
  hipLaunchKernelGGL(gn_cl_merge_kernel, dim3(groups, batch, nlevels), dim3(kThreads), 0, st, P);
  hipLaunchKernelGGL(gn_cl_apply_kernel, dim3(chunks), dim3(kThreads), 0, st, P);
  return launch_status();
}

int orp_affine_act_multi_cl(const orp_norm_level* levels, int nlevels, int batch, int channels, const float* coef, int relu,
                            const uint32_t* bound_in, int nsets, int per_set, uint32_t* slot_out, void* stream) {
  GnClParams P;
  const int chunks = fill_cl(levels, nlevels, batch, channels, 1, P);
  if (const int rc = fill_status(chunks)) return rc;
  if (!coef || (bound_in && (!slot_out || nsets <= 0 || per_set <= 0))) return ORP_EINVAL;
  P.eps = 0.f; P.relu = relu ? 1 : 0; P.partial = nullptr; P.stats = nullptr; P.pmax = nullptr; P.amax = nullptr;
  hipLaunchKernelGGL(affine_cl_kernel, dim3(chunks), dim3(kThreads), 0, (hipStream_t)stream, P, reinterpret_cast<const float2*>(coef),
                     bound_in, slot_out, nsets, per_set);
  return launch_status();
}

int orp_groupnorm_act_multi_cl(const orp_norm_level* levels, const float* const* gammas_host, const float* const* betas_host,
                               int nlevels, int batch, int channels, int groups, float eps, int relu, void* workspace,
                               size_t workspace_bytes, void* stream) {
  return gn_cl_impl(levels, gammas_host, betas_host, nlevels, batch, channels, groups, eps, relu, nullptr, nullptr, 0, workspace,
                    workspace_bytes, stream);
}

int orp_groupnorm_act_multi_cl_amax(const orp_norm_level* levels, const float* const* gammas_host, const float* const* betas_host,
                                    int nlevels, int batch, int channels, int groups, float eps, int relu, const int* slots_host,
                                    uint32_t* amax_out, int nslots, void* workspace, size_t workspace_bytes, void* stream) {
  if (!amax_out) return ORP_EINVAL;
  return gn_cl_impl(levels, gammas_host, betas_host, nlevels, batch, channels, groups, eps, relu, slots_host, amax_out, nslots,
                    workspace, workspace_bytes, stream);
}

int orp_groupnorm_act_multi_train(const orp_norm_level* levels, const float* const* gammas_host,
                                  const float* const* betas_host, int nlevels, int batch, int channels, int groups,
                                  float eps, int relu, float* stats, void* workspace, size_t workspace_bytes, void* stream) {
  return gn_nchw_forward(levels, gammas_host, betas_host, nlevels, batch, channels, groups, eps, relu, true, stats, workspace,
                         workspace_bytes, stream);
}

size_t orp_groupnorm_backward_workspace_bytes(const orp_norm_level* levels, int nlevels, int batch, int channels, int groups) {
  GnParams P;
  const int chunks = fill(levels, nlevels, batch, channels, groups, P);
  return chunks > 0 ? sizeof(float4) * (size_t)chunks * (size_t)(channels / groups) + 256 : 256;
}

int orp_groupnorm_act_multi_backward(const orp_norm_level* levels, const float* const* grad_outputs_host,
                                     float* const* grad_inputs_host, const float* const* gammas_host,
                                     const float* const* betas_host, float* const* dgammas_host, float* const* dbetas_host,
                                     int nlevels, int batch, int channels, int groups, int relu, const float* stats,
                                     void* workspace, size_t workspace_bytes, void* stream) {
  GnParams P;
  const int chunks = fill(levels, nlevels, batch, channels, groups, P);
  if (const int rc = fill_status(chunks)) return rc;
  if (!grad_outputs_host || !grad_inputs_host || !gammas_host || !betas_host || !dgammas_host ||
      !dbetas_host || !stats)
    return ORP_EINVAL;
  const int cg = channels / groups;
  if (!workspace || workspace_bytes < sizeof(float4) * (size_t)chunks * cg) return ORP_EWORKSPACE;
  if (!set_affine(P, gammas_host, betas_host, nlevels)) return ORP_EINVAL;
  for (int i = 0; i < nlevels; i++) {
    if (!grad_outputs_host[i] || !grad_inputs_host[i]) return ORP_EINVAL;
    P.dy[i] = grad_outputs_host[i]; P.dx[i] = grad_inputs_host[i];
  }
  for (int i = nlevels; i < kGnMaxLevels; i++) { P.dy[i] = nullptr; P.dx[i] = nullptr; }
  P.eps = 0.f; P.relu = relu;
  P.partial = nullptr;
  P.stats = reinterpret_cast<float2*>(const_cast<float*>(stats));
  P.bpart = reinterpret_cast<float4*>(workspace);
  hipStream_t st = (hipStream_t)stream;
  hipLaunchKernelGGL(gn_bwd_partial_kernel, dim3(chunks), dim3(kThreads), 0, st, P);
  hipLaunchKernelGGL(gn_bwd_apply_kernel, dim3(chunks), dim3(kThreads), 0, st, P);
  for (int i = 0; i < nlevels; i++) {
    bool first = true;
    for (int j = 0; j < i; j++) if (gammas_host[j] == gammas_host[i]) first = false;
    if (!first || !dgammas_host[i] || !dbetas_host[i]) continue;
    hipLaunchKernelGGL(gn_bwd_param_kernel, dim3((channels + 255) / 256), dim3(256), 0, st, P, gammas_host[i], dgammas_host[i],
                       dbetas_host[i]);
  }
  return launch_status();
}

int orp_groupnorm_act_multi(const orp_norm_level* levels, int nlevels, int batch, int channels, int groups,
                            const float* gamma, const float* beta, float eps, int relu, void* workspace,
                            size_t workspace_bytes, void* stream) {
  if (nlevels <= 0 || nlevels > kGnMaxLevels) return ORP_EINVAL;
  const float* g[kGnMaxLevels]; const float* b[kGnMaxLevels];
  for (int i = 0; i < nlevels; i++) { g[i] = gamma; b[i] = beta; }
  return orp_groupnorm_act_multi_ex(levels, g, b, nlevels, batch, channels, groups, eps, relu, workspace, workspace_bytes,
                                    stream);
}

int orp_affine_act(const float* x, const float* residual, const float* scale, const float* shift, float* y, int batch,
                   int channels, int hw, int relu, void* stream) {
  if (!x || !scale || !shift || !y || batch <= 0 || channels <= 0 || hw <= 0) return ORP_EINVAL;
  if ((long)batch * channels > 65535L * 1024) return ORP_ETOOBIG;
  hipLaunchKernelGGL(affine_act_kernel, dim3(plane_blocks(hw), batch * channels), dim3(kThreads), 0, (hipStream_t)stream, x, residual,
                     scale, shift, y, channels, hw, relu);
  return launch_status();
}

int orp_affine2_act(const float* x, const float* residual, const float* scale, const float* shift, const float* scale2,
                    const float* shift2, float* y, int batch, int channels, int hw, int relu, void* stream) {
  if (!x || !residual || !scale || !shift || !scale2 || !shift2 || !y || batch <= 0 || channels <= 0 || hw <= 0) return ORP_EINVAL;
  if ((long)batch * channels > 65535L * 1024) return ORP_ETOOBIG;
  hipLaunchKernelGGL(affine2_act_kernel, dim3(plane_blocks(hw), batch * channels), dim3(kThreads), 0, (hipStream_t)stream, x, residual,
                     scale, shift, scale2, shift2, y, channels, hw, relu);
  return launch_status();
}

int orp_affine_relu_maxpool(const float* x, const float* scale, const float* shift, float* y, int batch, int channels,
                            int height, int width, void* stream) {
  if (!x || !scale || !shift || !y || x == y || batch <= 0 || channels <= 0 || height <= 0 || width <= 0) return ORP_EINVAL;
  if ((long)batch * channels > 65535L || (long)height * width >= (1L << 31)) return ORP_ETOOBIG;
  const int ho = (height - 1) / 2 + 1, wo = (width - 1) / 2 + 1;
  const int nq = (wo + 1) / 2;
  const long items = (long)nq * ((ho + kPoolRows - 1) / kPoolRows);
  long bx = (items + kThreads - 1) / kThreads;
  if (bx > 65535) bx = 65535;
  const bool vec = (width & 3) == 0 && ((uintptr_t)x & 15) == 0 && ((uintptr_t)y & 7) == 0;
  const dim3 grid((unsigned)bx, batch * channels);
  if (vec)
    hipLaunchKernelGGL(affine_relu_maxpool_kernel<true>, grid, dim3(kThreads), 0, (hipStream_t)stream, x, scale, shift, y, channels,
                       height, width, ho, wo, nq, (int)items);
  else
    hipLaunchKernelGGL(affine_relu_maxpool_kernel<false>, grid, dim3(kThreads), 0, (hipStream_t)stream, x, scale, shift, y, channels,
                       height, width, ho, wo, nq, (int)items);
  return launch_status();
}

static size_t td_stats_offset(size_t chunks) { return (sizeof(float2) * chunks + 255) & ~(size_t)255; }

size_t orp_fpn_topdown_workspace_bytes(const orp_norm_level* levels, int nlevels, int batch, int channels, int groups) {
  GnParams P;
  const int chunks = fill(levels, nlevels, batch, channels, groups, P);
  if (chunks <= 0) return 256;
  return td_stats_offset(chunks) + sizeof(float2) * (size_t)nlevels * batch * groups;
}

int orp_fpn_topdown_nhwc(const orp_norm_level* levels, const float* const* gammas_host, const float* const* betas_host,
                         int nlevels, int batch, int channels, int groups, float eps, uint32_t* amax_out, void* workspace,
                         size_t workspace_bytes, void* stream) {
  GnParams P;
  if (!levels || nlevels <= 0 || nlevels > kTdMaxLevels) return ORP_EINVAL;
  const int chunks = fill(levels, nlevels, batch, channels, groups, P);
  if (const int rc = fill_status(chunks)) return rc;
  if (!gammas_host || !betas_host) return ORP_EINVAL;
  if (channels % 32 != 0 || 32 % (channels / groups) != 0 || batch > 65535) return ORP_EINVAL;
  const size_t nspan = (size_t)nlevels * batch * groups;
  const size_t stat_off = td_stats_offset(chunks);
  if (!workspace || ((uintptr_t)workspace & 7) != 0 || workspace_bytes < stat_off + sizeof(float2) * nspan) return ORP_EWORKSPACE;
  TdLevels T;
  int bx = 0;
  if (!set_affine(P, gammas_host, betas_host, nlevels)) return ORP_EINVAL;
  for (int i = 0; i < nlevels; i++) {
    if (levels[i].output == levels[i].input) return ORP_EINVAL;
    if (i + 1 < nlevels && (levels[i].height != 2 * levels[i + 1].height || levels[i].width != 2 * levels[i + 1].width))
      return ORP_EINVAL;
    T.out[i] = levels[i].output; T.width[i] = levels[i].width;
    T.bx0[i] = bx;
    bx += (P.lv[i].hw + 32 * kTdTiles - 1) / (32 * kTdTiles);
  }
  for (int i = nlevels; i <= kTdMaxLevels; i++) T.bx0[i] = 0x7fffffff;
  for (int i = nlevels; i < kTdMaxLevels; i++) { T.out[i] = T.out[0]; T.width[i] = T.width[0]; }
  T.stats = reinterpret_cast<float2*>(reinterpret_cast<char*>(workspace) + stat_off);
  T.amax = amax_out;
  P.eps = eps; P.relu = 0;
  P.partial = reinterpret_cast<float2*>(workspace);
  P.stats = nullptr;
  hipStream_t st = (hipStream_t)stream;
  hipLaunchKernelGGL(gn_stats_kernel, dim3(chunks), dim3(kThreads), 0, st, P);
  hipLaunchKernelGGL(gn_merge_kernel, dim3(batch * groups, nlevels), dim3(kThreads), 0, st, P, T);
  hipLaunchKernelGGL(fpn_topdown_nhwc_kernel, dim3(bx, channels / 32, batch), dim3(kThreads), 0, st, P, T);
  return launch_status();
}

int orp_bias_act_multi(const orp_bias_level* levels_host, int nlevels, int batch, int channels, const float* bias,
                       const float* sub, int relu, void* stream) {
  if (!levels_host || nlevels <= 0 || nlevels > kMaxLevels || batch <= 0 || channels <= 0) return ORP_EINVAL;
  if ((long)batch * channels > 65535L) return ORP_ETOOBIG;
  BiasParams P;
  P.nlev = nlevels; P.C = channels; P.relu = relu ? 1 : 0; P.bias = bias; P.sub = sub;
  int bx = 0;
  for (int i = 0; i < nlevels; i++) {
    const orp_bias_level& lv = levels_host[i];
    if (!lv.input || !lv.output || lv.height <= 0 || lv.width <= 0 || (lv.output2 && !sub)) return ORP_EINVAL;
    BiasLevel& L = P.lv[i];
    L.x = lv.input; L.res = lv.residual; L.y = lv.output; L.y2 = lv.output2;
    L.hw = lv.height * lv.width;
    L.bx0 = bx;
    bx += plane_blocks(L.hw);
  }
  for (int i = nlevels; i < kMaxLevels; i++) { P.lv[i] = P.lv[0]; P.lv[i].bx0 = 0x7fffffff; }
  hipLaunchKernelGGL(bias_act_multi_kernel, dim3(bx, batch * channels), dim3(kThreads), 0, (hipStream_t)stream, P);
  return launch_status();
}

}
```

orientedreppoints_amd/mmdet_models/resnet.py:

```python
import torch
import torch.nn as nn

from .layers import build_conv_layer, build_norm_layer, constant_init, kaiming_init
from .registry import BACKBONES


class Bottleneck(nn.Module):
    expansion = 4

    def __init__(self, inplanes, planes, stride=1, dilation=1, downsample=None, style='pytorch',
                 norm_cfg=dict(type='BN'), dcn=None):
        super(Bottleneck, self).__init__()
        assert style in ['pytorch', 'caffe']
        assert dcn is None or isinstance(dcn, dict)
        if style == 'pytorch':
            conv1_stride, conv2_stride = 1, stride
        else:
            conv1_stride, conv2_stride = stride, 1
        self.conv1 = nn.Conv2d(inplanes, planes, kernel_size=1, stride=conv1_stride, bias=False)
        self.add_module('bn1', build_norm_layer(norm_cfg, planes)[1])
        self.with_dcn = dcn is not None
        fallback_on_stride = False
        if self.with_dcn:
            fallback_on_stride = dcn.pop('fallback_on_stride', False)
            dcn = dict(dcn)
            if 'modulated' in dcn:
                dcn.setdefault('type', 'DCNv2' if dcn.pop('modulated') else 'DCN')
            dcn.setdefault('type', 'DCN')
        use_dcn = self.with_dcn and not fallback_on_stride
        self.conv2 = build_conv_layer(dcn if use_dcn else None, planes, planes, kernel_size=3, stride=conv2_stride,
                                      padding=dilation, dilation=dilation, bias=False)
        self.conv2_is_dcn = use_dcn
        self.add_module('bn2', build_norm_layer(norm_cfg, planes)[1])
        self.conv3 = nn.Conv2d(planes, planes * self.expansion, kernel_size=1, bias=False)
        self.add_module('bn3', build_norm_layer(norm_cfg, planes * self.expansion)[1])
        self.relu = nn.ReLU(inplace=True)
        self.downsample = downsample

    def _fused_ok(self, x):
        return (not torch.is_grad_enabled()) and x.is_cuda and x.dtype == torch.float32 and \
            isinstance(self.bn1, nn.BatchNorm2d) and not self.bn1.training and not self.bn3.training

    def _downsample_norm_fusable(self):
        from .. import switches
        on = getattr(self, 'fuse_downsample_norm', None)
        if on is None:
            on = switches.BN_DOWNSAMPLE_FUSE
        ds = self.downsample
        return bool(on) and isinstance(ds, nn.Sequential) and len(ds) == 2 and isinstance(ds[0], nn.Conv2d) and \
            isinstance(ds[1], nn.BatchNorm2d) and not ds[1].training

    def _conv1x1_fusable(self):
        from .. import switches
        on = getattr(self, 'fuse_conv1x1', None)
        if on is None:
            on = switches.BN_CONV1X1_FUSE
        return bool(on)

    def _forward_fused(self, x):
        from ..mmdet_ops.fused_norm import bn_act, conv1x1_bn_act
        fuse = self._conv1x1_fusable()

        def conv_bn_act(t, conv, bn, **kw):
            if fuse:
                return conv1x1_bn_act(t, conv, bn, **kw)
            return bn_act(conv(t).contiguous(), bn, **kw)
        out = conv_bn_act(x, self.conv1, self.bn1, relu=True)
        out = bn_act(self.conv2(out).contiguous(), self.bn2, relu=True)
        if self._downsample_norm_fusable():
            return conv_bn_act(out, self.conv3, self.bn3, residual=self.downsample[0](x).contiguous(),
                               residual_bn=self.downsample[1], relu=True)
        if self.downsample is not None:
            identity = bn_act(self.downsample[0](x).contiguous(), self.downsample[1], relu=False)
        else:
            identity = x.contiguous()
        return conv_bn_act(out, self.conv3, self.bn3, residual=identity, relu=True)

    def forward(self, x):
        if self._fused_ok(x):
            return self._forward_fused(x)
        identity = x
        out = self.relu(self.bn1(self.conv1(x)))
        out = self.relu(self.bn2(self.conv2(out)))
        out = self.bn3(self.conv3(out))
        if self.downsample is not None:
            identity = self.downsample(x)
        out += identity
        return self.relu(out)


@BACKBONES.register_module
class ResNet(nn.Module):
    arch_settings = {50: (Bottleneck, (3, 4, 6, 3)), 101: (Bottleneck, (3, 4, 23, 3)), 152: (Bottleneck, (3, 8, 36, 3))}

    def __init__(self, depth, in_channels=3, num_stages=4, strides=(1, 2, 2, 2), dilations=(1, 1, 1, 1),
                 out_indices=(0, 1, 2, 3), style='pytorch', frozen_stages=-1, conv_cfg=None,
                 norm_cfg=dict(type='BN', requires_grad=True), norm_eval=True, dcn=None,
                 stage_with_dcn=(False, False, False, False), gcb=None, stage_with_gcb=None, gen_attention=None,
                 stage_with_gen_attention=None, with_cp=False, zero_init_residual=True):
        super(ResNet, self).__init__()
        if depth not in self.arch_settings:
            raise KeyError('invalid depth {} for resnet'.format(depth))
        assert gcb is None and gen_attention is None, 'context / attention blocks are not part of the DOTA configs'
        assert conv_cfg is None, 'the backbone convolutions are stock nn.Conv2d (dcn= selects the deformable conv2)'
        self.dcn = dict(dcn) if dcn is not None else None
        self.stage_with_dcn = tuple(stage_with_dcn) if stage_with_dcn is not None else (False,) * num_stages
        if dcn is not None:
            assert len(self.stage_with_dcn) == num_stages
        self.depth, self.num_stages, self.out_indices = depth, num_stages, out_indices
        self.frozen_stages, self.norm_eval = frozen_stages, norm_eval
        self.zero_init_residual = zero_init_residual
        block, stage_blocks = self.arch_settings[depth]
        self.conv1 = nn.Conv2d(in_channels, 64, kernel_size=7, stride=2, padding=3, bias=False)
        self.add_module('bn1', build_norm_layer(norm_cfg, 64)[1])
        self.relu = nn.ReLU(inplace=True)
        self.maxpool = nn.MaxPool2d(kernel_size=3, stride=2, padding=1)
        inplanes = 64
        self.res_layers = []
        for i, num_blocks in enumerate(stage_blocks[:num_stages]):
            planes = 64 * 2 ** i
            stride, dilation = strides[i], dilations[i]
            downsample = None
            if stride != 1 or inplanes != planes * block.expansion:
                downsample = nn.Sequential(
                    nn.Conv2d(inplanes, planes * block.expansion, kernel_size=1, stride=stride, bias=False),
                    build_norm_layer(norm_cfg, planes * block.expansion)[1])
            stage_dcn = self.dcn if (self.dcn is not None and self.stage_with_dcn[i]) else None
            layers = [block(inplanes, planes, stride, dilation, downsample, style, norm_cfg, stage_dcn)]
            inplanes = planes * block.expansion
            for _ in range(1, num_blocks):
                layers.append(block(inplanes, planes, 1, dilation, None, style, norm_cfg, stage_dcn))
            name = 'layer{}'.format(i + 1)
            self.add_module(name, nn.Sequential(*layers))
            self.res_layers.append(name)
        self._freeze_stages()
        self.feat_dim = inplanes

    def _freeze_stages(self):
        if self.frozen_stages >= 0:
            self.bn1.eval()
            for m in [self.conv1, self.bn1]:
                for param in m.parameters():
                    param.requires_grad = False
        for i in range(1, self.frozen_stages + 1):
            m = getattr(self, 'layer{}'.format(i))
            m.eval()
            for param in m.parameters():
                param.requires_grad = False

    def init_weights(self, pretrained=None):
        if isinstance(pretrained, str):
            import os
            import warnings
            path = pretrained
            if '://' in pretrained:
                name = pretrained.split('://', 1)[1].replace('/', '_')
                root = os.environ.get('ORP_PRETRAINED_DIR', '')
                path = os.path.join(root, name + '.pth') if root else ''
            if path and os.path.isfile(path):
                sd = torch.load(path, map_location='cpu')
                sd = sd.get('state_dict', sd)
                missing, unexpected = self.load_state_dict(sd, strict=False)
                unexpected = [k for k in unexpected if not k.startswith('fc.')]
                if missing or unexpected:
                    warnings.warn('ResNet.init_weights(%r): missing keys %s, unexpected keys %s'
                                  % (pretrained, list(missing)[:8], unexpected[:8]))
                return
            warnings.warn('ResNet.init_weights: pretrained=%r was NOT loaded (no such file%s); the backbone keeps its '
                          'random initialisation, frozen_stages=%d of it frozen'
                          % (pretrained, '' if '://' not in pretrained else '; set ORP_PRETRAINED_DIR', self.frozen_stages))
        for m in self.modules():
            if isinstance(m, nn.Conv2d):
                kaiming_init(m)
            elif isinstance(m, (nn.BatchNorm2d, nn.GroupNorm)):
                constant_init(m, 1)
        if self.dcn is not None:
            for m in self.modules():
                if isinstance(m, Bottleneck) and hasattr(m.conv2, 'conv_offset'):
                    constant_init(m.conv2.conv_offset, 0)
        if self.zero_init_residual:
            for m in self.modules():
                if isinstance(m, Bottleneck):
                    constant_init(m.bn3, 0)

    def _stem_pool_fusable(self):
        from .. import switches
        on = getattr(self, 'fuse_stem_pool', None)
        if on is None:
            on = switches.STEM_POOL_FUSE

        def pair(v):
            return tuple(v) if isinstance(v, (tuple, list)) else (v, v)
        mp = self.maxpool
        return bool(on) and type(mp) is nn.MaxPool2d and pair(mp.kernel_size) == (3, 3) and pair(mp.stride) == (2, 2) and \
            pair(mp.padding) == (1, 1) and pair(mp.dilation) == (1, 1) and not mp.ceil_mode and not mp.return_indices

    def forward(self, x):
        if (not torch.is_grad_enabled()) and x.is_cuda and x.dtype == torch.float32 and \
                isinstance(self.bn1, nn.BatchNorm2d) and not self.bn1.training:
            from ..mmdet_ops.fused_norm import bn_act, bn_relu_maxpool
            if self._stem_pool_fusable():
                x = bn_relu_maxpool(self.conv1(x).contiguous(), self.bn1)
            else:
                x = self.maxpool(bn_act(self.conv1(x).contiguous(), self.bn1, relu=True))
        else:
            x = self.maxpool(self.relu(self.bn1(self.conv1(x))))
        outs = []
        for i, name in enumerate(self.res_layers):
            x = getattr(self, name)(x)
            if i in self.out_indices:
                outs.append(x)
        return tuple(outs)

    def train(self, mode=True):
        super(ResNet, self).train(mode)
        self._freeze_stages()
        if mode and self.norm_eval:
            for m in self.modules():
                if isinstance(m, nn.modules.batchnorm._BatchNorm):
                    m.eval()
```

orientedreppoints_amd/mmdet_ops/fused_norm.py:

```python
import ctypes

import torch

from .. import _lib, _packcache


class _NormLevel(ctypes.Structure):
    _fields_ = [("input", ctypes.c_void_p), ("output", ctypes.c_void_p), ("height", ctypes.c_int),
                ("width", ctypes.c_int)]


def _norm_levels(ins, outs):
    levels = (_NormLevel * len(ins))()
    for i, (x, y) in enumerate(zip(ins, outs)):
        levels[i] = _NormLevel(x.data_ptr(), y.data_ptr() if y is not None else None, x.size(2), x.size(3))
    return levels


def _gn_modules(gn, n, who):
    gns = list(gn) if isinstance(gn, (list, tuple)) else [gn] * n
    if len(gns) != n or any(g.num_groups != gns[0].num_groups or g.eps != gns[0].eps for g in gns):
        raise ValueError(who + ": one GroupNorm per tensor, equal num_groups / eps")
    index, distinct, owner = {}, [], []
    for g in gns:
        if id(g) not in index:
            index[id(g)] = len(distinct)
            distinct.append(g)
        owner.append(index[id(g)])
    return gns, distinct, owner


def _ptrs(tensors, owner=None):
    owner = range(len(tensors)) if owner is None else owner
    return (ctypes.c_void_p * len(owner))(*[tensors[k].data_ptr() for k in owner])


def _param_ptrs(weights, biases, owner):
    gs = [w.detach().float().contiguous() for w in weights]
    bs = [b.detach().float().contiguous() for b in biases]
    return _ptrs(gs, owner), _ptrs(bs, owner), gs, bs


def _affine_ptrs(mods, owner):
    return _param_ptrs([m.weight for m in mods], [m.bias for m in mods], owner)


def group_norm_act_multi(xs, gn, relu=True, inplace=True, nhwc=None):
    L = _lib.lib()
    x0 = xs[0]
    B, C = x0.size(0), x0.size(1)
    gns, mods, owner = _gn_modules(gn, len(xs), "group_norm_act_multi")
    ins, outs = [], []
    for x in xs:
        if not (x.is_cuda and x.dtype == torch.float32 and x.dim() == 4 and x.size(0) == B and x.size(1) == C):
            raise ValueError("group_norm_act_multi expects fp32 CUDA [B,C,H,W] tensors with equal B and C")
        x = x.detach().contiguous()
        ins.append(x); outs.append(x if inplace else torch.empty_like(x))
    levels = _norm_levels(ins, outs)
    gam, bet, _gs, _bs = _affine_ptrs(mods, owner)
    nbytes = L.orp_groupnorm_workspace_bytes(levels, len(xs), B, C, gns[0].num_groups)
    ws = _lib.workspace(x0.device, nbytes)
    if nhwc is not None:
        if nhwc not in ('only', 'both') or C % 32 != 0 or 32 % (C // gns[0].num_groups) != 0:
            raise ValueError("group_norm_act_multi(nhwc=...): 'only' | 'both', channels % 32 == 0, 32 % (channels / groups) == 0")
        cl = [torch.empty(x.shape, dtype=torch.float32, device=x.device, memory_format=torch.channels_last) for x in ins]
        cl_ptrs = _ptrs(cl)
        if nhwc == 'only':
            for i in range(len(xs)):
                levels[i].output = None
        with torch.cuda.device(x0.device):
            rc = L.orp_groupnorm_act_multi_nhwc(levels, gam, bet, cl_ptrs, len(xs), B, C, gns[0].num_groups, float(gns[0].eps),
                                                1 if relu else 0, _lib.ptr(ws), ws.numel(), _lib.stream_of(x0))
        _lib.check(rc, "orp_groupnorm_act_multi_nhwc")
        return cl if nhwc == 'only' else (outs, cl)
    with torch.cuda.device(x0.device):
        rc = L.orp_groupnorm_act_multi_ex(levels, gam, bet, len(xs), B, C, gns[0].num_groups, float(gns[0].eps),
                                          1 if relu else 0, _lib.ptr(ws), ws.numel(), _lib.stream_of(x0))
    _lib.check(rc, "orp_groupnorm_act_multi_ex")
    return outs


def group_norm_act_multi_cl(xs, gn, relu=True, inplace=True, amax_slots=None):
    L = _lib.lib()
    x0 = xs[0]
    B, C = x0.size(0), x0.size(1)
    gns, mods, owner = _gn_modules(gn, len(xs), "group_norm_act_multi_cl")
    G = gns[0].num_groups
    if 1024 % C != 0 or C % G != 0 or (C // G) % 4 != 0:
        raise ValueError("group_norm_act_multi_cl: 1024 % channels == 0 and (channels / groups) % 4 == 0")
    ins = [x.detach() for x in xs]
    for x in ins:
        if not (x.is_cuda and x.dtype == torch.float32 and x.dim() == 4 and x.size(0) == B and x.size(1) == C and _is_cl(x)):
            raise ValueError("group_norm_act_multi_cl expects channels-last fp32 CUDA [B,C,H,W] tensors with equal B and C")
    outs = ins if inplace else [torch.empty_like(x, memory_format=torch.channels_last) for x in ins]
    levels = _norm_levels(ins, outs)
    gam, bet, _gs, _bs = _affine_ptrs(mods, owner)
    nbytes = L.orp_groupnorm_cl_workspace_bytes(levels, len(xs), B, C, G)
    ws = _lib.workspace(x0.device, nbytes)
    if amax_slots is not None and not _ranges_wanted():
        amax_slots, no_ranges = None, True
    else:
        no_ranges = False
    if amax_slots is not None:
        slots = (ctypes.c_int * len(xs))(*[int(v) for v in amax_slots])
        bits = torch.empty(max(int(v) for v in amax_slots) + 1, dtype=torch.int32, device=x0.device)
        with torch.cuda.device(x0.device):
            rc = L.orp_groupnorm_act_multi_cl_amax(levels, gam, bet, len(xs), B, C, G, float(gns[0].eps), 1 if relu else 0, slots,
                                                   bits.data_ptr(), bits.numel(), _lib.ptr(ws), ws.numel(), _lib.stream_of(x0))
        _lib.check(rc, "orp_groupnorm_act_multi_cl_amax")
        return outs, bits
    with torch.cuda.device(x0.device):
        rc = L.orp_groupnorm_act_multi_cl(levels, gam, bet, len(xs), B, C, G, float(gns[0].eps), 1 if relu else 0,
                                          _lib.ptr(ws), ws.numel(), _lib.stream_of(x0))
    _lib.check(rc, "orp_groupnorm_act_multi_cl")
    return (outs, None) if no_ranges else outs


_affine_cache = _packcache.new_cache("bn_affine")


def _bn_affine(bn):
    def st(t):
        return _packcache.tensor_state(t) if t is not None else None
    state = (st(bn.weight), st(bn.bias), st(bn.running_mean), st(bn.running_var), float(bn.eps))
    hit = _affine_cache.get(bn, state)
    if hit is None:
        with torch.no_grad():
            rstd = torch.rsqrt(bn.running_var.float() + bn.eps)
            w = bn.weight.float() if bn.weight is not None else torch.ones_like(rstd)
            b = bn.bias.float() if bn.bias is not None else torch.zeros_like(rstd)
            scale = (w * rstd).contiguous()
            shift = (b - bn.running_mean.float() * scale).contiguous()
        hit = _affine_cache.put(bn, state, (scale, shift))
    return _lib.keep_for_graph(hit[0]), _lib.keep_for_graph(hit[1])


def bn_act(x, bn, residual=None, relu=True, residual_bn=None):
    if not (x.is_cuda and x.dtype == torch.float32 and x.dim() == 4 and x.is_contiguous()):
        raise ValueError("bn_act expects a contiguous fp32 CUDA [B,C,H,W] tensor")
    if residual is not None and not (residual.shape == x.shape and residual.is_contiguous()
                                     and residual.dtype == torch.float32):
        raise ValueError("bn_act: residual must match x")
    if residual_bn is not None and residual is None:
        raise ValueError("bn_act: residual_bn without a residual")
    scale, shift = _bn_affine(bn)
    B, C, H, W = x.shape
    if residual_bn is not None:
        scale2, shift2 = _bn_affine(residual_bn)
        with torch.cuda.device(x.device):
            rc = _lib.lib().orp_affine2_act(_lib.ptr(x), _lib.ptr(residual), _lib.ptr(scale), _lib.ptr(shift), _lib.ptr(scale2),
                                            _lib.ptr(shift2), _lib.ptr(x), B, C, H * W, 1 if relu else 0, _lib.stream_of(x))
        _lib.check(rc, "orp_affine2_act")
        return x
    with torch.cuda.device(x.device):
        rc = _lib.lib().orp_affine_act(_lib.ptr(x), _lib.ptr(residual), _lib.ptr(scale), _lib.ptr(shift), _lib.ptr(x),
                                       B, C, H * W, 1 if relu else 0, _lib.stream_of(x))
    _lib.check(rc, "orp_affine_act")
    return x


_packed_1x1_t = _packcache.new_cache("conv1x1_bn_weight")


def _transposed_1x1_weight(weight):
    w = weight.detach()
    state = _packcache.tensor_state(w)
    hit = _packed_1x1_t.get(weight, state)
    if hit is None:
        hit = _packed_1x1_t.put(weight, state, w.float().reshape(w.size(0), w.size(1)).t().contiguous())
    return _lib.keep_for_graph(hit)


def conv1x1_bn_act_ok(x, conv, bn):
    w = conv.weight
    return bool(isinstance(conv, torch.nn.Conv2d) and isinstance(bn, torch.nn.BatchNorm2d) and not bn.training and
                x.is_cuda and x.dtype == torch.float32 and x.dim() == 4 and w.dtype == torch.float32 and w.dim() == 4 and
                w.size(2) == 1 and w.size(3) == 1 and x.size(1) == w.size(1) and conv.bias is None and
                tuple(conv.stride) == (1, 1) and tuple(conv.padding) == (0, 0) and tuple(conv.dilation) == (1, 1) and
                conv.groups == 1 and x.size(2) * x.size(3) > 0 and _lib.lib().orp_conv1x1_bn_act_ok(w.size(1), w.size(0)))


def conv1x1_bn_act(x, conv, bn, residual=None, residual_bn=None, relu=True, force=False):
    if residual_bn is not None and residual is None:
        raise ValueError("conv1x1_bn_act: residual_bn without a residual")
    L = _lib.lib()
    fused = conv1x1_bn_act_ok(x, conv, bn) and (residual_bn is None or not residual_bn.training)
    if fused and not force:
        fused = bool(L.orp_conv1x1_bn_act_pays(x.size(1), conv.weight.size(0), x.size(2) * x.size(3), x.size(0),
                                                1 if residual is not None else 0))
    if not fused:
        return bn_act(conv(x).contiguous(), bn, residual=residual, relu=relu, residual_bn=residual_bn)
    x = x.detach().contiguous()
    B, cin, H, W = x.shape
    cout = conv.weight.size(0)
    if residual is not None:
        residual = residual.detach()
        if not (tuple(residual.shape) == (B, cout, H, W) and residual.is_contiguous() and residual.dtype == torch.float32):
            raise ValueError("conv1x1_bn_act: residual must be a contiguous fp32 tensor of the output's shape")
    wt = _transposed_1x1_weight(conv.weight)
    scale, shift = _bn_affine(bn)
    scale2, shift2 = _bn_affine(residual_bn) if residual_bn is not None else (None, None)
    y = torch.empty((B, cout, H, W), dtype=torch.float32, device=x.device)
    with torch.cuda.device(x.device):
        rc = L.orp_conv1x1_bn_act(_lib.ptr(x), _lib.ptr(wt), _lib.ptr(scale), _lib.ptr(shift), _lib.ptr(residual),
                                  _lib.ptr(scale2), _lib.ptr(shift2), _lib.ptr(y), B, cin, cout, H * W, 1 if relu else 0,
                                  _lib.stream_of(x))
    _lib.check(rc, "orp_conv1x1_bn_act")
    return y


def bn_relu_maxpool(x, bn):
    if not (x.is_cuda and x.dtype == torch.float32 and x.dim() == 4 and x.is_contiguous()):
        raise ValueError("bn_relu_maxpool expects a contiguous fp32 CUDA [B,C,H,W] tensor")
    scale, shift = _bn_affine(bn)
    B, C, H, W = x.shape
    y = torch.empty((B, C, (H - 1) // 2 + 1, (W - 1) // 2 + 1), dtype=torch.float32, device=x.device)
    with torch.cuda.device(x.device):
        rc = _lib.lib().orp_affine_relu_maxpool(_lib.ptr(x), _lib.ptr(scale), _lib.ptr(shift), _lib.ptr(y), B, C, H, W,
                                                _lib.stream_of(x))
    _lib.check(rc, "orp_affine_relu_maxpool")
    return y


def fpn_topdown_ok(xs, gns):
    x0, g0 = xs[0], gns[0]
    B, C = x0.size(0), x0.size(1)
    if not (1 <= len(xs) <= 4 and len(gns) == len(xs) and C % 32 == 0 and C % g0.num_groups == 0 and 32 % (C // g0.num_groups) == 0):
        return False
    for i, (x, g) in enumerate(zip(xs, gns)):
        if not (x.is_cuda and x.dtype == torch.float32 and x.dim() == 4 and x.size(0) == B and x.size(1) == C and
                isinstance(g, torch.nn.GroupNorm) and g.affine and g.num_groups == g0.num_groups and g.eps == g0.eps):
            return False
        if i and (xs[i - 1].size(2) != 2 * x.size(2) or xs[i - 1].size(3) != 2 * x.size(3)):
            return False
    return True


def fpn_topdown_cl(xs, gns, amax=True):
    if not fpn_topdown_ok(xs, gns):
        raise ValueError("fpn_topdown_cl: see fpn_topdown_ok")
    L = _lib.lib()
    x0 = xs[0]
    B, C = x0.size(0), x0.size(1)
    n = len(xs)
    gns, mods, owner = _gn_modules(gns, n, "fpn_topdown_cl")
    ins = [x.detach().contiguous() for x in xs]
    outs = [torch.empty(x.shape, dtype=torch.float32, device=x.device, memory_format=torch.channels_last) for x in ins]
    levels = _norm_levels(ins, outs)
    gam, bet, _gs, _bs = _affine_ptrs(mods, owner)
    bits = torch.empty(1, dtype=torch.int32, device=x0.device) if (amax and _ranges_wanted()) else None
    nbytes = L.orp_fpn_topdown_workspace_bytes(levels, n, B, C, gns[0].num_groups)
    ws = _lib.workspace(x0.device, nbytes)
    with torch.cuda.device(x0.device):
        rc = L.orp_fpn_topdown_nhwc(levels, gam, bet, n, B, C, gns[0].num_groups, float(gns[0].eps),
                                    bits.data_ptr() if bits is not None else None, _lib.ptr(ws), ws.numel(), _lib.stream_of(x0))
    _lib.check(rc, "orp_fpn_topdown_nhwc")
    return outs, bits


class _BiasLevel(ctypes.Structure):
    _fields_ = [("input", ctypes.c_void_p), ("residual", ctypes.c_void_p), ("output", ctypes.c_void_p),
                ("output2", ctypes.c_void_p), ("height", ctypes.c_int), ("width", ctypes.c_int)]


def bias_act_multi(xs, bias, relu=False, residuals=None, sub=None):
    x0 = xs[0]
    B, C = x0.size(0), x0.size(1)
    levels = (_BiasLevel * len(xs))()
    ys, zs = [], []
    keep = []
    for i, x in enumerate(xs):
        if not (x.is_cuda and x.dtype == torch.float32 and x.dim() == 4 and x.size(0) == B and x.size(1) == C):
            raise ValueError("bias_act_multi expects fp32 CUDA [B,C,H,W] tensors with equal B and C")
        x = x.detach().contiguous()
        r = None
        if residuals is not None:
            r = residuals[i].detach().contiguous()
            if r.shape != x.shape or r.dtype != torch.float32:
                raise ValueError("bias_act_multi: residual must match x")
            keep.append(r)
        z = torch.empty_like(x) if sub is not None else None
        ys.append(x); zs.append(z)
        levels[i] = _BiasLevel(x.data_ptr(), r.data_ptr() if r is not None else None, x.data_ptr(),
                               z.data_ptr() if z is not None else None, x.size(2), x.size(3))
    b = bias.detach().float().contiguous() if bias is not None else None
    s = sub.detach().float().reshape(-1).contiguous() if sub is not None else None
    if (b is not None and b.numel() != C) or (s is not None and s.numel() != C):
        raise ValueError("bias_act_multi: bias / sub must have C elements")
    with torch.cuda.device(x0.device):
        rc = _lib.lib().orp_bias_act_multi(levels, len(xs), B, C, _lib.ptr(b), _lib.ptr(s), 1 if relu else 0,
                                           _lib.stream_of(x0))
    _lib.check(rc, "orp_bias_act_multi")
    return (ys, zs) if sub is not None else ys


_packed_1x1 = _packcache.new_cache("conv1x1_weight")


def _packed_1x1_weight(weight):
    w = weight.detach()
    state = _packcache.tensor_state(w)
    hit = _packed_1x1.get(weight, state)
    if hit is not None:
        return _lib.keep_for_graph(hit)
    cout, cin = w.size(0), w.size(1)
    w2 = w.float().reshape(cout, cin).contiguous()
    packed = torch.empty((_lib.lib().orp_conv1x1_packed_floats(cin),), dtype=torch.float32, device=w.device)
    with torch.cuda.device(w.device):
        _lib.check(_lib.lib().orp_conv1x1_pack_weight(_lib.ptr(w2), cout, cin, _lib.ptr(packed), _lib.stream_of(w2)),
                   "orp_conv1x1_pack_weight")
    return _lib.keep_for_graph(_packed_1x1.put(weight, state, packed))


def conv1x1_ok(conv, x):
    w = conv.weight
    return bool(x.is_cuda and x.dtype == torch.float32 and w.dim() == 4 and w.size(2) == 1 and w.size(3) == 1 and
                tuple(conv.stride) == (1, 1) and tuple(conv.padding) == (0, 0) and conv.groups == 1 and
                _lib.lib().orp_conv1x1_ok(w.size(1), w.size(0)))


def conv1x1_multi(xs, conv, relu=False, residuals=None, sub=None):
    x0 = xs[0]
    B, cin = x0.size(0), x0.size(1)
    cout = conv.weight.size(0)
    packed = _packed_1x1_weight(conv.weight)
    levels = (_BiasLevel * len(xs))()
    ys, zs, keep = [], [], []
    for i, x in enumerate(xs):
        if not (x.is_cuda and x.dtype == torch.float32 and x.dim() == 4 and x.size(0) == B and x.size(1) == cin):
            raise ValueError("conv1x1_multi expects fp32 CUDA [B,Cin,H,W] tensors with equal B and Cin")
        x = x.detach().contiguous()
        y = torch.empty((B, cout, x.size(2), x.size(3)), dtype=torch.float32, device=x.device)
        r = None
        if residuals is not None:
            r = residuals[i].detach().contiguous()
            if r.shape != y.shape or r.dtype != torch.float32:
                raise ValueError("conv1x1_multi: residual must match the output")
        z = torch.empty_like(y) if sub is not None else None
        keep += [x, r]
        ys.append(y); zs.append(z)
        levels[i] = _BiasLevel(x.data_ptr(), r.data_ptr() if r is not None else None, y.data_ptr(),
                               z.data_ptr() if z is not None else None, x.size(2), x.size(3))
    b = conv.bias.detach().float().contiguous() if conv.bias is not None else None
    s = sub.detach().float().reshape(-1).contiguous() if sub is not None else None
    if s is not None and s.numel() != cout:
        raise ValueError("conv1x1_multi: sub must have Cout elements")
    with torch.cuda.device(x0.device):
        rc = _lib.lib().orp_conv1x1_multi(levels, len(xs), B, cin, cout, _lib.ptr(packed), _lib.ptr(b), _lib.ptr(s),
                                          1 if relu else 0, _lib.stream_of(x0))
    _lib.check(rc, "orp_conv1x1_multi")
    return (ys, zs) if sub is not None else ys


SMALL_LEVEL_POSITIONS = 1024


def conv3x3_multi(xs, conv, split_k=False):
    import torch.nn.functional as F
    from .deform_conv import _packed_weight
    convs = list(conv) if isinstance(conv, (list, tuple)) else [conv] * len(xs)
# ... 504 lines not shown
```

orientedreppoints_amd/switches.py:

```python
import os


def _on(name, default='1'):
    return os.environ.get(name, default) == '1'


TOWER_SPLIT = _on('ORP_TOWER_SPLIT')
FPN_SPLIT = _on('ORP_FPN_SPLIT')
TOWER_GN_FUSE = _on('ORP_TOWER_GN_FUSE')
BN_DOWNSAMPLE_FUSE = _on('ORP_BN_DOWNSAMPLE_FUSE')
BN_CONV1X1_FUSE = _on('ORP_BN_CONV1X1_FUSE')
STEM_POOL_FUSE = _on('ORP_STEM_POOL_FUSE')
FPN_TOPDOWN_FUSE = _on('ORP_FPN_TOPDOWN_FUSE')
TRAIN_SPLIT = _on('ORP_TRAIN_SPLIT')
DETERMINISTIC = _on('ORP_DETERMINISTIC', '0')
```

Before: 371.6 images/s.

## Add fused 3x3 conv+BN+ReLU MFMA kernel for ResNet bottlenecks using fp16 split planes

```diff
diff --git a/include/orp_hip.h b/include/orp_hip.h
--- a/include/orp_hip.h
+++ b/include/orp_hip.h
@@ -270,6 +270,22 @@
                        const float* scale2, const float* shift2, float* y, int batch, int c_in, int c_out, int hw, int relu,
                        void* stream);
 
+int orp_conv1x1_bn_act_range(const float* x, const float* weight_t, const float* scale, const float* shift, const float* residual,
+                             const float* scale2, const float* shift2, float* y, int batch, int c_in, int c_out, int hw, int relu,
+                             uint32_t* range_out, void* stream);
+int orp_affine_act_range(const float* x, const float* residual, const float* scale, const float* shift, float* y, int batch,
+                         int channels, int hw, int relu, uint32_t* range_out, void* stream);
+
+int orp_conv3x3_bn_act_ok(int c_in, int c_out);
+int orp_conv3x3_bn_act_pays(int c_in, int c_out, int height, int width, int batch);
+int orp_conv3x3_bn_act_tile(int c_in, int c_out, int height, int width, int batch, int* tile_h, int* tile_w, int* waves_pos,
+                            int* waves_ch);
+size_t orp_conv3x3_bn_packed_bytes(int c_in, int c_out);
+int orp_conv3x3_bn_pack_weight(const float* weight, int c_in, int c_out, void* packed, void* stream);
+int orp_conv3x3_bn_act(const float* x, const void* weight_packed, const float* scale, const float* shift, const uint32_t* range_in,
+                       float* y, int batch, int c_in, int c_out, int height, int width, int relu, void* stream);
+
+
 int orp_conv3x3_small_ok(int c_in, int c_out);
 int orp_conv3x3_small_multi(const orp_norm_level* levels_host, int nlevels, int batch, int c_in, int c_out,
                             const float* weight_packed, void* stream);
diff --git a/orientedreppoints_amd/_lib.py b/orientedreppoints_amd/_lib.py
--- a/orientedreppoints_amd/_lib.py
+++ b/orientedreppoints_amd/_lib.py
@@ -101,6 +101,14 @@
     "orp_conv1x1_bn_act_pays": (_i, [_i, _i, _i, _i, _i]),
     "orp_conv1x1_bn_act_tile": (_i, [_i, _i, _i, _i, _vp, _vp]),
     "orp_conv1x1_bn_act": (_i, [_vp, _vp, _vp, _vp, _vp, _vp, _vp, _vp, _i, _i, _i, _i, _i, _vp]),
+    "orp_conv1x1_bn_act_range": (_i, [_vp, _vp, _vp, _vp, _vp, _vp, _vp, _vp, _i, _i, _i, _i, _i, _vp, _vp]),
+    "orp_affine_act_range": (_i, [_vp, _vp, _vp, _vp, _vp, _i, _i, _i, _i, _vp, _vp]),
+    "orp_conv3x3_bn_act_ok": (_i, [_i, _i]),
+    "orp_conv3x3_bn_act_pays": (_i, [_i, _i, _i, _i, _i]),
+    "orp_conv3x3_bn_act_tile": (_i, [_i, _i, _i, _i, _i, _vp, _vp, _vp, _vp]),
+    "orp_conv3x3_bn_packed_bytes": (_sz, [_i, _i]),
+    "orp_conv3x3_bn_pack_weight": (_i, [_vp, _i, _i, _vp, _vp]),
+    "orp_conv3x3_bn_act": (_i, [_vp, _vp, _vp, _vp, _vp, _vp, _i, _i, _i, _i, _i, _i, _vp]),
     "orp_pp_select_scratch_bytes": (_sz, [_i, _i, _i]),
     "orp_pp_select": (_i, [_vp, _i, _i, _vp, _i, _i, _vp, _vp, _sz, _vp]),
     "orp_pp_gather": (_i, [_vp, _vp, _i, _i, _vp, _vp, _vp, _i, _vp, _vp, _vp, _vp, _vp]),
diff --git a/orientedreppoints_amd/build.py b/orientedreppoints_amd/build.py
--- a/orientedreppoints_amd/build.py
+++ b/orientedreppoints_amd/build.py
@@ -32,6 +32,7 @@
     ("orp_conv_small.hip", []),
     ("orp_conv1x1.hip", []),
     ("orp_conv1x1_bn.hip", []),
+    ("orp_conv3x3_bn.hip", []),
     ("orp_dcn.hip", []),
     ("orp_dcn_split.hip", ["-ffp-contract=off"]),
     ("orp_conv_split.hip", []),
diff --git a/orientedreppoints_amd/csrc/orp_conv1x1_bn.hip b/orientedreppoints_amd/csrc/orp_conv1x1_bn.hip
--- a/orientedreppoints_amd/csrc/orp_conv1x1_bn.hip
+++ b/orientedreppoints_amd/csrc/orp_conv1x1_bn.hip
@@ -3,6 +3,8 @@
 
 #include "../../include/orp_hip.h"
 #include "orp_affine.hpp"
+#include "orp_range.hpp"
+#include "orp_launch.hpp"
 
 namespace {
 
@@ -20,9 +22,10 @@
   float* y;
   int cin, cout, hw, relu;
   int ntm, ntn;
+  unsigned* range;
 };
 
-template <int WM, int WN, bool VEC, int MODE>
+template <int WM, int WN, bool VEC, int MODE, bool RANGE = false>
 __global__ void __launch_bounds__(kThreads, 2)
 conv1x1_bn_act_kernel(const Args P) {
   constexpr int BM = 64 * WM, BN = 64 * WN;
@@ -151,6 +154,7 @@
   __builtin_amdgcn_sched_barrier(0);
   mma();
 
+  unsigned rmax = 0u;
 #pragma unroll
   for (int mi = 0; mi < WM; mi++) {
 #pragma unroll
@@ -178,10 +182,22 @@
           if (MODE == 0) t = affine_act(v, av[q], bv[q], P.relu);
           else if (MODE == 1) t = affine_res_act(v, av[q], bv[q], rv[mi][ni][r], P.relu);
           else t = affine_res_act(v, av[q], bv[q], affine_act(rv[mi][ni][r], a2v[q], b2v[q], 0), P.relu);
-          if (chg < cout && p < hw) P.y[(plane0 + chg + q) * hw + p] = t;
+          if (chg < cout && p < hw) {
+            P.y[(plane0 + chg + q) * hw + p] = t;
+            if (RANGE) rmax = max(rmax, orp::range_bits(t));
+          }
         }
       }
     }
+  }
+  if (RANGE) {
+#pragma unroll
+    for (int o = 32; o > 0; o >>= 1) rmax = max(rmax, (unsigned)__shfl_xor((int)rmax, o, 64));
+    unsigned* red = reinterpret_cast<unsigned*>(Ws);
+    __syncthreads();
+    if (lane == 0) red[wave] = rmax;
+    __syncthreads();
+    if (tid == 0) orp::range_raise(P.range, max(max(red[0], red[1]), max(red[2], red[3])));
   }
 }
 
@@ -206,7 +222,11 @@
 }
 template <int WM, int WN>
 void launch(const Args& A, int batch, bool vec, hipStream_t st) {
-  if (!A.res) launch_mode<WM, WN, 0>(A, batch, vec, st);
+  if (A.range) {
+    const dim3 grid((unsigned)((long)A.ntm * A.ntn * batch));
+    if (vec) hipLaunchKernelGGL((conv1x1_bn_act_kernel<WM, WN, true, 0, true>), grid, dim3(kThreads), 0, st, A);
+    else hipLaunchKernelGGL((conv1x1_bn_act_kernel<WM, WN, false, 0, true>), grid, dim3(kThreads), 0, st, A);
+  } else if (!A.res) launch_mode<WM, WN, 0>(A, batch, vec, st);
   else if (!A.scale2) launch_mode<WM, WN, 1>(A, batch, vec, st);
   else launch_mode<WM, WN, 2>(A, batch, vec, st);
 }
@@ -246,9 +266,10 @@
   return 0;
 }
 
-int orp_conv1x1_bn_act(const float* x, const float* weight_t, const float* scale, const float* shift, const float* residual,
-                       const float* scale2, const float* shift2, float* y, int batch, int c_in, int c_out, int hw, int relu,
-                       void* stream) {
+int orp_conv1x1_bn_act_range(const float* x, const float* weight_t, const float* scale, const float* shift, const float* residual,
+                             const float* scale2, const float* shift2, float* y, int batch, int c_in, int c_out, int hw, int relu,
+                             uint32_t* range_out, void* stream) {
+  if (range_out && residual) return ORP_EINVAL;
   if (!x || !weight_t || !scale || !shift || !y || batch <= 0 || hw <= 0 || !orp_conv1x1_bn_act_ok(c_in, c_out)) return ORP_EINVAL;
   if ((scale2 != nullptr) != (shift2 != nullptr) || (scale2 && !residual) || (const float*)y == x || (const float*)y == residual)
     return ORP_EINVAL;
@@ -258,9 +279,14 @@
   A.x = x; A.wt = weight_t; A.scale = scale; A.shift = shift; A.res = residual; A.scale2 = scale2; A.shift2 = shift2; A.y = y;
   A.cin = c_in; A.cout = c_out; A.hw = hw; A.relu = relu ? 1 : 0;
   A.ntm = (c_out + t.bm - 1) / t.bm; A.ntn = (hw + t.bn - 1) / t.bn;
+  A.range = range_out;
   if ((long)A.ntm * A.ntn * batch >= (1L << 31)) return ORP_ETOOBIG;
   const bool vec = (hw & 3) == 0 && ((uintptr_t)x & 15) == 0;
   hipStream_t st = (hipStream_t)stream;
+  if (range_out) {
+    hipError_t fe = orp::fill_async(range_out, 0, sizeof(uint32_t), st);
+    if (fe != hipSuccess) return (int)fe;
+  }
   if (t.bm == 128) launch<2, 2>(A, batch, vec, st);
   else if (t.bn == 128) launch<1, 2>(A, batch, vec, st);
   else launch<1, 1>(A, batch, vec, st);
@@ -268,4 +294,10 @@
   return e == hipSuccess ? ORP_OK : (int)e;
 }
 
-}
+int orp_conv1x1_bn_act(const float* x, const float* weight_t, const float* scale, const float* shift, const float* residual,
+                       const float* scale2, const float* shift2, float* y, int batch, int c_in, int c_out, int hw, int relu,
+                       void* stream) {
+  return orp_conv1x1_bn_act_range(x, weight_t, scale, shift, residual, scale2, shift2, y, batch, c_in, c_out, hw, relu, nullptr, stream);
+}
+
+}
diff --git a/orientedreppoints_amd/csrc/orp_conv3x3_bn.hip b/orientedreppoints_amd/csrc/orp_conv3x3_bn.hip
--- /dev/null
+++ b/orientedreppoints_amd/csrc/orp_conv3x3_bn.hip
@@ -0,0 +1,279 @@
+#include <hip/hip_runtime.h>
+#include <stdint.h>
+
+#include "../../include/orp_hip.h"
+#include "orp_affine.hpp"
+#include "orp_range.hpp"
+#include "orp_launch.hpp"
+#include "orp_dcn_split.hpp"
+
+namespace {
+
+typedef float floatx16 __attribute__((ext_vector_type(16)));
+typedef _Float16 h8 __attribute__((ext_vector_type(8)));
+typedef _Float16 h2 __attribute__((ext_vector_type(2)));
+
+constexpr int kThreads = 512;
+constexpr int TW = 16;
+constexpr int HWID = TW + 2;
+constexpr int NCH = 4;
+
+struct Args {
+  const float* x;
+  const uint16_t* planes;
+  size_t plane_stride;
+  const float* wscale;
+  const unsigned* range;
+  const float* scale; const float* shift;
+  float* y;
+  int H, W, relu, tiles_x, tiles_per_image;
+};
+
+template <int C, int WM, int MT>
+struct Cfg {
+  static constexpr int WN = 8 / WM;
+  static_assert(WN * 32 == C, "a wave owns 32 output channels");
+  static constexpr int TH = 2 * WM * MT;
+  static constexpr int ROWS = (TH + 2) * HWID;
+  static constexpr int ASTR = C + 8;
+  static constexpr size_t smem = (size_t)2 * ROWS * ASTR * 2;
+};
+
+template <int C, int WM, int MT>
+__global__ void __launch_bounds__(kThreads)
+conv3x3_bn_act_kernel(const Args P) {
+  using K = Cfg<C, WM, MT>;
+  constexpr int ASTR = K::ASTR, PLANE = K::ROWS * ASTR;
+  extern __shared__ __attribute__((aligned(16))) unsigned char smem[];
+  uint16_t* sA = reinterpret_cast<uint16_t*>(smem);
+
+  const int tid = threadIdx.x, lane = tid & 63, wave = tid >> 6;
+  const int tile = blockIdx.x;
+  const int img = tile / P.tiles_per_image, tt = tile - img * P.tiles_per_image;
+  const int trow = tt / P.tiles_x;
+  const int y0 = trow * K::TH, x0 = (tt - trow * P.tiles_x) * TW;
+  const int H = P.H, W = P.W;
+  const size_t hw = (size_t)H * W;
+
+  const int kx = orp::range_exp(*P.range);
+  const float sx = orp::range_scale(kx);
+  const int kxw = kx + orp::range_exp_of(*P.wscale);
+
+  const int wn = wave % K::WN, wm = wave / K::WN;
+  const int n_wave = wn * 32;
+  const int mrow = lane & 31, kg = lane >> 5;
+  const uint16_t* wp = P.planes + ((size_t)kg * C + n_wave + mrow) * 8;
+  constexpr size_t wblk = (size_t)2 * C * 8;
+  auto load_b = [&](int ph, int j, h8 (&b)[2]) {
+    const uint16_t* a = wp + ((size_t)ph * NCH + j) * wblk;
+#pragma unroll
+    for (int pl = 0; pl < 2; pl++) b[pl] = *reinterpret_cast<const h8*>(a + (size_t)pl * P.plane_stride);
+  };
+  h8 bq[NCH][2];
+#pragma unroll
+  for (int j = 0; j < NCH; j++) load_b(0, j, bq[j]);
+  __builtin_amdgcn_sched_barrier(0);
+
+  {
+    const int px = lane & 15, cq = lane >> 4;
+    const float* xb = P.x + (size_t)img * C * hw + (size_t)((wave * 4 + cq) * 2) * hw;
+    constexpr int NPB = (K::ROWS + 15) / 16, G = C == 64 ? 7 : C == 128 ? 4 : 3, NCB = C / 64;
+#pragma unroll 1
+    for (int pb0 = 0; pb0 < NPB; pb0 += G) {
+      float v[G][NCB][2];
+      bool in[G];
+#pragma unroll
+      for (int g = 0; g < G; g++) {
+        const int h = (pb0 + g) * 16 + px;
+        const int hy = h / HWID, hx = h - hy * HWID;
+        const int yy = y0 - 1 + hy, xx = x0 - 1 + hx;
+        in[g] = h < K::ROWS && yy >= 0 && yy < H && xx >= 0 && xx < W;
+        const float* src = xb + (in[g] ? (size_t)yy * W + xx : (size_t)0);
+#pragma unroll
+        for (int cb = 0; cb < NCB; cb++) {
+          v[g][cb][0] = src[(size_t)(cb * 64) * hw];
+          v[g][cb][1] = src[(size_t)(cb * 64 + 1) * hw];
+        }
+      }
+#pragma unroll
+      for (int g = 0; g < G; g++)
+#pragma unroll
+        for (int cb = 0; cb < NCB; cb++) { asm volatile("" : "+v"(v[g][cb][0])); asm volatile("" : "+v"(v[g][cb][1])); }
+#pragma unroll
+      for (int g = 0; g < G; g++) {
+        const int h = (pb0 + g) * 16 + px;
+#pragma unroll
+        for (int cb = 0; cb < NCB; cb++) {
+          const float s0 = in[g] ? v[g][cb][0] * sx : 0.f, s1 = in[g] ? v[g][cb][1] * sx : 0.f;
+          h2 hh, ll;
+          orp::range_split(s0, hh, ll, 0);
+          orp::range_split(s1, hh, ll, 1);
+          if (h < K::ROWS) {
+            uint16_t* dst = sA + (size_t)h * ASTR + cb * 64 + (wave * 4 + cq) * 2;
+            *reinterpret_cast<unsigned*>(dst) = __builtin_bit_cast(unsigned, hh);
+            *reinterpret_cast<unsigned*>(dst + PLANE) = __builtin_bit_cast(unsigned, ll);
+          }
+        }
+      }
+    }
+  }
+  __syncthreads();
+
+  auto tyx = [&](int m, int& ty, int& tx) { ty = m >> 4; tx = (m - 2 * ty) & 15; };
+  const uint16_t* abase[MT];
+#pragma unroll
+  for (int mt = 0; mt < MT; mt++) {
+    int ty, tx;
+    tyx((wm * MT + mt) * 32 + mrow, ty, tx);
+    abase[mt] = sA + (size_t)(ty * HWID + tx) * ASTR + 8 * kg;
+  }
+  auto a_off = [&](int ph) {
+    const int tap = ph / (C / 64), cb = ph - tap * (C / 64);
+    const int ki = tap / 3;
+    return (ki * HWID + tap - 3 * ki) * ASTR + cb * 64;
+  };
+  auto load_a = [&](int off, int j, h8 (&a)[MT][2]) {
+#pragma unroll
+    for (int mt = 0; mt < MT; mt++)
+#pragma unroll
+      for (int pl = 0; pl < 2; pl++) a[mt][pl] = *reinterpret_cast<const h8*>(abase[mt] + pl * PLANE + off + j * 16);
+  };
+
+  floatx16 acc[MT], side[MT];
+#pragma unroll
+  for (int mt = 0; mt < MT; mt++) { acc[mt] = floatx16{0}; side[mt] = floatx16{0}; }
+  constexpr int nphase = 9 * (C / 64);
+  h8 a[2][MT][2];
+  load_a(a_off(0), 0, a[0]);
+#pragma unroll 1
+  for (int ph = 0; ph < nphase; ph++) {
+    const int ph_n = ph + 1 < nphase ? ph + 1 : ph;
+    const int off = a_off(ph), off_n = a_off(ph_n);
+#pragma unroll
+    for (int j = 0; j < NCH; j++) {
+      if (j + 1 < NCH) load_a(off, j + 1, a[(j + 1) & 1]);
+      else             load_a(off_n, 0, a[0]);
+      __builtin_amdgcn_sched_barrier(0);
+#pragma unroll
+      for (int mt = 0; mt < MT; mt++) side[mt] = __builtin_amdgcn_mfma_f32_32x32x16_f16(bq[j][0], a[j & 1][mt][1], side[mt], 0, 0, 0);
+#pragma unroll
+      for (int mt = 0; mt < MT; mt++) side[mt] = __builtin_amdgcn_mfma_f32_32x32x16_f16(bq[j][1], a[j & 1][mt][0], side[mt], 0, 0, 0);
+#pragma unroll
+      for (int mt = 0; mt < MT; mt++) acc[mt] = __builtin_amdgcn_mfma_f32_32x32x16_f16(bq[j][0], a[j & 1][mt][0], acc[mt], 0, 0, 0);
+      __builtin_amdgcn_sched_barrier(0);
+      load_b(ph_n, j, bq[j]);
+      __builtin_amdgcn_sched_barrier(0);
+    }
+  }
+
+  float ca[16], cb_[16];
+#pragma unroll
+  for (int r = 0; r < 16; r++) {
+    const int ch = n_wave + (r & 3) + 8 * (r >> 2) + 4 * kg;
+    ca[r] = P.scale[ch]; cb_[r] = P.shift[ch];
+  }
+  float* yb = P.y + (size_t)img * C * hw;
+#pragma unroll
+  for (int mt = 0; mt < MT; mt++) {
+    int ty, tx;
+    tyx((wm * MT + mt) * 32 + mrow, ty, tx);
+    const int yy = y0 + ty, xx = x0 + tx;
+    if (yy < H && xx < W) {
+      float* o = yb + (size_t)yy * W + xx;
+#pragma unroll
+      for (int r = 0; r < 16; r++) {
+        const int ch = n_wave + (r & 3) + 8 * (r >> 2) + 4 * kg;
+        const float v = orp::range_unscale(acc[mt][r] + side[mt][r], kxw);
+        o[(size_t)ch * hw] = affine_act(v, ca[r], cb_[r], P.relu);
+      }
+    }
+  }
+}
+
+struct Layout { int wm, wn, mt, th; };
+
+bool layout_of(int c, Layout& l) {
+  if (c == 64) l = Layout{4, 2, 2, 16};
+  else if (c == 128) l = Layout{2, 4, 1, 4};
+  else if (c == 256) l = Layout{1, 8, 1, 2};
+  else return false;
+  return true;
+}
+
+template <int C, int WM, int MT>
+hipError_t launch(const Args& A, long tiles, hipStream_t st) {
+  using K = Cfg<C, WM, MT>;
+  struct Tag {};
+  hipError_t e = orp::set_max_dynamic_lds_once<Tag>(reinterpret_cast<const void*>(&conv3x3_bn_act_kernel<C, WM, MT>), K::smem);
+  if (e != hipSuccess) return e;
+  hipLaunchKernelGGL((conv3x3_bn_act_kernel<C, WM, MT>), dim3((unsigned)tiles), dim3(kThreads), K::smem, st, A);
+  return hipGetLastError();
+}
+
+}
+
+extern "C" {
+
+int orp_conv3x3_bn_act_ok(int c_in, int c_out) {
+  return (c_in == c_out && (c_in == 64 || c_in == 128 || c_in == 256)) ? 1 : 0;
+}
+
+size_t orp_conv3x3_bn_packed_bytes(int c_in, int c_out) {
+  return orp_conv3x3_bn_act_ok(c_in, c_out) ? (size_t)4 * c_in * c_out * 9 + 16 : 0;
+}
+
+int orp_conv3x3_bn_pack_weight(const float* weight, int c_in, int c_out, void* packed, void* stream) {
+  if (!weight || !packed || ((uintptr_t)packed & 15) || !orp_conv3x3_bn_act_ok(c_in, c_out)) return ORP_EINVAL;
+  uint16_t* planes = reinterpret_cast<uint16_t*>(packed);
+  const size_t n = (size_t)c_in * c_out * 9;
+  hipError_t e = orp_split::pack_planes16(weight, c_out, c_in, 9, planes, reinterpret_cast<float*>(planes + 2 * n), (hipStream_t)stream);
+  return e == hipSuccess ? ORP_OK : (int)e;
+}
+
+int orp_conv3x3_bn_act_tile(int c_in, int c_out, int height, int width, int batch, int* tile_h, int* tile_w, int* waves_pos,
+                            int* waves_ch) {
+  Layout l;
+  if (!orp_conv3x3_bn_act_ok(c_in, c_out) || height <= 0 || width <= 0 || batch <= 0 || !layout_of(c_in, l)) return 0;
+  if (tile_h) *tile_h = l.th;
+  if (tile_w) *tile_w = TW;
+  if (waves_pos) *waves_pos = l.wm;
+  if (waves_ch) *waves_ch = l.wn;
+  return 1;
+}
+
+int orp_conv3x3_bn_act_pays(int c_in, int c_out, int height, int width, int batch) {
+  if (!orp_conv3x3_bn_act_ok(c_in, c_out) || height <= 0 || width <= 0 || batch <= 0) return 0;
+  static const struct { int c, side_min, side_max, batch; } paid[] = {
+      {64, 256, 384, 1},  {64, 256, 256, 2},
+      {128, 128, 192, 1}, {128, 128, 128, 2},
+      {256, 64, 96, 1},   {256, 64, 64, 2},
+  };
+  for (const auto& s : paid)
+    if (s.c == c_in && s.batch == batch && height >= s.side_min && height <= s.side_max && width >= s.side_min && width <= s.side_max)
+      return 1;
+  return 0;
+}
+
+int orp_conv3x3_bn_act(const float* x, const void* weight_packed, const float* scale, const float* shift, const uint32_t* range_in,
+                       float* y, int batch, int c_in, int c_out, int height, int width, int relu, void* stream) {
+  Layout l;
+  if (!x || !weight_packed || ((uintptr_t)weight_packed & 15) || !scale || !shift || !range_in || !y || (const float*)y == x || batch <= 0 || height <= 0 || width <= 0 ||
+      !orp_conv3x3_bn_act_ok(c_in, c_out) || !layout_of(c_in, l))
+    return ORP_EINVAL;
+  Args A;
+  A.x = x; A.scale = scale; A.shift = shift; A.y = y; A.range = range_in;
+  A.planes = reinterpret_cast<const uint16_t*>(weight_packed);
+  A.plane_stride = (size_t)c_out * c_in * 9;
+  A.wscale = reinterpret_cast<const float*>(A.planes + 2 * A.plane_stride);
+  A.H = height; A.W = width; A.relu = relu ? 1 : 0;
+  A.tiles_x = (width + TW - 1) / TW;
+  const long tpi = (long)A.tiles_x * ((height + l.th - 1) / l.th);
+  if (tpi * batch >= (1L << 31) || (long)height * width >= (1L << 31)) return ORP_ETOOBIG;
+  A.tiles_per_image = (int)tpi;
+  hipStream_t st = (hipStream_t)stream;
+  hipError_t e = c_in == 64 ? launch<64, 4, 2>(A, tpi * batch, st)
+               : c_in == 128 ? launch<128, 2, 1>(A, tpi * batch, st) : launch<256, 1, 1>(A, tpi * batch, st);
+  return e == hipSuccess ? ORP_OK : (int)e;
+}
+
+}
diff --git a/orientedreppoints_amd/csrc/orp_dcn_split.hip b/orientedreppoints_amd/csrc/orp_dcn_split.hip
--- a/orientedreppoints_amd/csrc/orp_dcn_split.hip
+++ b/orientedreppoints_amd/csrc/orp_dcn_split.hip
@@ -761,11 +761,9 @@
   return reinterpret_cast<const float*>(reinterpret_cast<const uint16_t*>(packed + 2 * n) + 5 * n);
 }
 
-hipError_t pack_planes(const float* weight, int c_out, int c_in, int taps, uint16_t* planes, hipStream_t st) {
+hipError_t pack_planes16(const float* weight, int c_out, int c_in, int taps, uint16_t* planes16, float* tail, hipStream_t st) {
   const long total = (long)c_out * c_in * taps;
   int blocks = (int)((total + 255) / 256); if (blocks > 4096) blocks = 4096;
-  hipLaunchKernelGGL(pack_planes_kernel, dim3(blocks), dim3(256), 0, st, weight, c_out, c_in, taps, planes);
-  float* tail = reinterpret_cast<float*>(planes + 5 * total);
   unsigned* amax = reinterpret_cast<unsigned*>(tail + 1);
   hipError_t e = orp::fill_async(amax, 0, sizeof(unsigned), st);
   if (e != hipSuccess) return e;
@@ -774,8 +772,15 @@
   for (int i = 0; i < kAbsMaxT; i++) { M.x[i] = weight; M.n[i] = i == 0 ? (size_t)total : 0; M.slot[i] = 0; M.bx0[i] = i == 0 ? 0 : (int)nb; }
   M.bx0[kAbsMaxT] = (int)nb; M.count = 1;
   hipLaunchKernelGGL(absmax_kernel, dim3((int)nb), dim3(256), 0, st, M, amax);
-  hipLaunchKernelGGL(pack_planes16_kernel, dim3(blocks), dim3(256), 0, st, weight, c_out, c_in, taps, amax, planes + 3 * total, tail);
+  hipLaunchKernelGGL(pack_planes16_kernel, dim3(blocks), dim3(256), 0, st, weight, c_out, c_in, taps, amax, planes16, tail);
   return hipGetLastError();
+}
+
+hipError_t pack_planes(const float* weight, int c_out, int c_in, int taps, uint16_t* planes, hipStream_t st) {
+  const long total = (long)c_out * c_in * taps;
+  int blocks = (int)((total + 255) / 256); if (blocks > 4096) blocks = 4096;
+  hipLaunchKernelGGL(pack_planes_kernel, dim3(blocks), dim3(256), 0, st, weight, c_out, c_in, taps, planes);
+  return pack_planes16(weight, c_out, c_in, taps, planes + 3 * total, reinterpret_cast<float*>(planes + 5 * total), st);
 }
 
 static int g_halo = -1;
diff --git a/orientedreppoints_amd/csrc/orp_dcn_split.hpp b/orientedreppoints_amd/csrc/orp_dcn_split.hpp
--- a/orientedreppoints_amd/csrc/orp_dcn_split.hpp
+++ b/orientedreppoints_amd/csrc/orp_dcn_split.hpp
@@ -53,6 +53,7 @@
 const uint16_t* planes_of(const float* packed, int c_out, int c_in, int taps, int nprod);
 const float* wscale_of(const float* packed, int c_out, int c_in, int taps);
 hipError_t pack_planes(const float* weight , int c_out, int c_in, int taps, uint16_t* planes, hipStream_t st);
+hipError_t pack_planes16(const float* weight, int c_out, int c_in, int taps, uint16_t* planes16, float* tail, hipStream_t st);
 hipError_t launch(const Args& a, hipStream_t st);
 int set_amax_log(unsigned* log, int capacity_launches);
 
diff --git a/orientedreppoints_amd/csrc/orp_norm.hip b/orientedreppoints_amd/csrc/orp_norm.hip
--- a/orientedreppoints_amd/csrc/orp_norm.hip
+++ b/orientedreppoints_amd/csrc/orp_norm.hip
@@ -340,9 +340,11 @@
   }
 }
 
+template <bool RANGE>
 __global__ void __launch_bounds__(kThreads)
 affine_act_kernel(const float* __restrict__ x, const float* __restrict__ res, const float* __restrict__ scale,
-                  const float* __restrict__ shift, float* __restrict__ y, int C, int hw, int relu) {
+                  const float* __restrict__ shift, float* __restrict__ y, int C, int hw, int relu, unsigned* __restrict__ range) {
+  unsigned rmax = 0u;
   const int plane = blockIdx.y;
   const int c = plane % C;
   const float a = scale[c], b = shift[c];
@@ -358,11 +360,19 @@
       if (r4) { const float4 r = r4[i]; t.x += r.x; t.y += r.y; t.z += r.z; t.w += r.w; }
       if (relu) relu4(t);
       y4[i] = t;
+      if (RANGE) rmax = max(max(rmax, orp::range_bits(t.x)), max(orp::range_bits(t.y), max(orp::range_bits(t.z), orp::range_bits(t.w))));
     }
   } else {
     for (int i = blockIdx.x * blockDim.x + threadIdx.x; i < hw; i += gridDim.x * blockDim.x) {
-      y[base + i] = res ? affine_res_act(x[base + i], a, b, res[base + i], relu) : affine_act(x[base + i], a, b, relu);
-    }
+      const float t = res ? affine_res_act(x[base + i], a, b, res[base + i], relu) : affine_act(x[base + i], a, b, relu);
+      y[base + i] = t;
+      if (RANGE) rmax = max(rmax, orp::range_bits(t));
+    }
+  }
+  if (RANGE) {
+    __shared__ unsigned redm[4];
+    const unsigned mx = block_max(rmax, redm);
+    if (threadIdx.x == 0) orp::range_raise(range, mx);
   }
 }
 
@@ -1004,13 +1014,26 @@
                                     stream);
 }
 
+int orp_affine_act_range(const float* x, const float* residual, const float* scale, const float* shift, float* y, int batch,
+                         int channels, int hw, int relu, uint32_t* range_out, void* stream) {
+  if (!x || !scale || !shift || !y || batch <= 0 || channels <= 0 || hw <= 0) return ORP_EINVAL;
+  if ((long)batch * channels > 65535L * 1024) return ORP_ETOOBIG;
+  const dim3 grid(plane_blocks(hw), batch * channels);
+  if (range_out) {
+    hipError_t e = orp::fill_async(range_out, 0, sizeof(uint32_t), (hipStream_t)stream);
+    if (e != hipSuccess) return (int)e;
+    hipLaunchKernelGGL(affine_act_kernel<true>, grid, dim3(kThreads), 0, (hipStream_t)stream, x, residual, scale, shift, y, channels,
+                       hw, relu, range_out);
+  } else {
+    hipLaunchKernelGGL(affine_act_kernel<false>, grid, dim3(kThreads), 0, (hipStream_t)stream, x, residual, scale, shift, y, channels,
+                       hw, relu, (unsigned*)nullptr);
+  }
+  return launch_status();
+}
+
 int orp_affine_act(const float* x, const float* residual, const float* scale, const float* shift, float* y, int batch,
                    int channels, int hw, int relu, void* stream) {
-  if (!x || !scale || !shift || !y || batch <= 0 || channels <= 0 || hw <= 0) return ORP_EINVAL;
-  if ((long)batch * channels > 65535L * 1024) return ORP_ETOOBIG;
-  hipLaunchKernelGGL(affine_act_kernel, dim3(plane_blocks(hw), batch * channels), dim3(kThreads), 0, (hipStream_t)stream, x, residual,
-                     scale, shift, y, channels, hw, relu);
-  return launch_status();
+  return orp_affine_act_range(x, residual, scale, shift, y, batch, channels, hw, relu, nullptr, stream);
 }
 
 int orp_affine2_act(const float* x, const float* residual, const float* scale, const float* shift, const float* scale2,
diff --git a/orientedreppoints_amd/mmdet_models/resnet.py b/orientedreppoints_amd/mmdet_models/resnet.py
--- a/orientedreppoints_amd/mmdet_models/resnet.py
+++ b/orientedreppoints_amd/mmdet_models/resnet.py
@@ -57,16 +57,32 @@
             on = switches.BN_CONV1X1_FUSE
         return bool(on)
 
+    def _conv3x3_fusable(self):
+        from .. import switches
+        on = getattr(self, 'fuse_conv3x3', None)
+        if on is None:
+            on = switches.BN_CONV3X3_FUSE
+        return bool(on) and not self.conv2_is_dcn and isinstance(self.bn2, nn.BatchNorm2d) and not self.bn2.training
+
     def _forward_fused(self, x):
-        from ..mmdet_ops.fused_norm import bn_act, conv1x1_bn_act
+        from ..mmdet_ops.fused_norm import bn_act, conv1x1_bn_act, conv3x3_bn_act, conv3x3_bn_act_routed
         fuse = self._conv1x1_fusable()
 
         def conv_bn_act(t, conv, bn, **kw):
             if fuse:
                 return conv1x1_bn_act(t, conv, bn, **kw)
             return bn_act(conv(t).contiguous(), bn, **kw)
-        out = conv_bn_act(x, self.conv1, self.bn1, relu=True)
-        out = bn_act(self.conv2(out).contiguous(), self.bn2, relu=True)
+        force3 = bool(getattr(self, 'force_conv3x3', False))
+        fuse3 = False
+        if self._conv3x3_fusable() and tuple(self.conv1.stride) == (1, 1):
+            fuse3 = conv3x3_bn_act_routed(x, self.conv2, self.bn2, force3,
+                                          shape=(x.size(0), self.conv1.out_channels, x.size(2), x.size(3)))
+        if fuse3:
+            out, bits = conv_bn_act(x, self.conv1, self.bn1, relu=True, want_range=True)
+            out = conv3x3_bn_act(out, self.conv2, self.bn2, relu=True, force=force3, range_bits=bits)
+        else:
+            out = conv_bn_act(x, self.conv1, self.bn1, relu=True)
+            out = bn_act(self.conv2(out).contiguous(), self.bn2, relu=True)
         if self._downsample_norm_fusable():
             return conv_bn_act(out, self.conv3, self.bn3, residual=self.downsample[0](x).contiguous(),
                                residual_bn=self.downsample[1], relu=True)
diff --git a/orientedreppoints_amd/mmdet_ops/fused_norm.py b/orientedreppoints_amd/mmdet_ops/fused_norm.py
--- a/orientedreppoints_amd/mmdet_ops/fused_norm.py
+++ b/orientedreppoints_amd/mmdet_ops/fused_norm.py
@@ -135,7 +135,7 @@
     return _lib.keep_for_graph(hit[0]), _lib.keep_for_graph(hit[1])
 
 
-def bn_act(x, bn, residual=None, relu=True, residual_bn=None):
+def bn_act(x, bn, residual=None, relu=True, residual_bn=None, want_range=False):
     if not (x.is_cuda and x.dtype == torch.float32 and x.dim() == 4 and x.is_contiguous()):
         raise ValueError("bn_act expects a contiguous fp32 CUDA [B,C,H,W] tensor")
     if residual is not None and not (residual.shape == x.shape and residual.is_contiguous()
@@ -143,8 +143,17 @@
         raise ValueError("bn_act: residual must match x")
     if residual_bn is not None and residual is None:
         raise ValueError("bn_act: residual_bn without a residual")
+    if want_range and residual_bn is not None:
+        raise ValueError("bn_act: want_range with residual_bn")
     scale, shift = _bn_affine(bn)
     B, C, H, W = x.shape
+    if want_range:
+        bits = torch.empty(1, dtype=torch.int32, device=x.device)
+        with torch.cuda.device(x.device):
+            rc = _lib.lib().orp_affine_act_range(_lib.ptr(x), _lib.ptr(residual), _lib.ptr(scale), _lib.ptr(shift), _lib.ptr(x),
+                                                 B, C, H * W, 1 if relu else 0, _lib.ptr(bits), _lib.stream_of(x))
+        _lib.check(rc, "orp_affine_act_range")
+        return x, bits
     if residual_bn is not None:
         scale2, shift2 = _bn_affine(residual_bn)
         with torch.cuda.device(x.device):
@@ -180,16 +189,18 @@
                 conv.groups == 1 and x.size(2) * x.size(3) > 0 and _lib.lib().orp_conv1x1_bn_act_ok(w.size(1), w.size(0)))
 
 
-def conv1x1_bn_act(x, conv, bn, residual=None, residual_bn=None, relu=True, force=False):
+def conv1x1_bn_act(x, conv, bn, residual=None, residual_bn=None, relu=True, force=False, want_range=False):
     if residual_bn is not None and residual is None:
         raise ValueError("conv1x1_bn_act: residual_bn without a residual")
+    if want_range and residual is not None:
+        raise ValueError("conv1x1_bn_act: want_range with a residual")
     L = _lib.lib()
     fused = conv1x1_bn_act_ok(x, conv, bn) and (residual_bn is None or not residual_bn.training)
     if fused and not force:
         fused = bool(L.orp_conv1x1_bn_act_pays(x.size(1), conv.weight.size(0), x.size(2) * x.size(3), x.size(0),
                                                 1 if residual is not None else 0))
     if not fused:
-        return bn_act(conv(x).contiguous(), bn, residual=residual, relu=relu, residual_bn=residual_bn)
+        return bn_act(conv(x).contiguous(), bn, residual=residual, relu=relu, residual_bn=residual_bn, want_range=want_range)
     x = x.detach().contiguous()
     B, cin, H, W = x.shape
     cout = conv.weight.size(0)
@@ -201,11 +212,77 @@
     scale, shift = _bn_affine(bn)
     scale2, shift2 = _bn_affine(residual_bn) if residual_bn is not None else (None, None)
     y = torch.empty((B, cout, H, W), dtype=torch.float32, device=x.device)
+    if want_range:
+        bits = torch.empty(1, dtype=torch.int32, device=x.device)
+        with torch.cuda.device(x.device):
+            rc = L.orp_conv1x1_bn_act_range(_lib.ptr(x), _lib.ptr(wt), _lib.ptr(scale), _lib.ptr(shift), None, None, None,
+                                            _lib.ptr(y), B, cin, cout, H * W, 1 if relu else 0, _lib.ptr(bits), _lib.stream_of(x))
+        _lib.check(rc, "orp_conv1x1_bn_act_range")
+        return y, bits
     with torch.cuda.device(x.device):
         rc = L.orp_conv1x1_bn_act(_lib.ptr(x), _lib.ptr(wt), _lib.ptr(scale), _lib.ptr(shift), _lib.ptr(residual),
                                   _lib.ptr(scale2), _lib.ptr(shift2), _lib.ptr(y), B, cin, cout, H * W, 1 if relu else 0,
                                   _lib.stream_of(x))
     _lib.check(rc, "orp_conv1x1_bn_act")
+    return y
+
+
+def conv3x3_bn_act_ok(x, conv, bn, shape=None):
+    w = getattr(conv, 'weight', None)
+    shape = tuple(x.shape) if shape is None else tuple(shape)
+    return bool(type(conv) is torch.nn.Conv2d and isinstance(bn, torch.nn.BatchNorm2d) and not bn.training and
+                x.is_cuda and x.dtype == torch.float32 and len(shape) == 4 and w.dtype == torch.float32 and w.dim() == 4 and
+                w.size(2) == 3 and w.size(3) == 3 and shape[1] == w.size(1) and conv.bias is None and
+                tuple(conv.stride) == (1, 1) and tuple(conv.padding) == (1, 1) and tuple(conv.dilation) == (1, 1) and
+                conv.groups == 1 and shape[0] * shape[2] * shape[3] > 0 and _lib.lib().orp_conv3x3_bn_act_ok(w.size(1), w.size(0)))
+
+
+def conv3x3_bn_act_routed(x, conv, bn, force=False, shape=None):
+    if not conv3x3_bn_act_ok(x, conv, bn, shape):
+        return False
+    B, _c, H, W = tuple(x.shape) if shape is None else tuple(shape)
+    return bool(force or _lib.lib().orp_conv3x3_bn_act_pays(conv.weight.size(1), conv.weight.size(0), H, W, B))
+
+
+def conv3x3_bn_act_tile(cin, cout, H, W, B):
+    v = [ctypes.c_int() for _ in range(4)]
+    if not _lib.lib().orp_conv3x3_bn_act_tile(int(cin), int(cout), int(H), int(W), int(B), *[ctypes.byref(t) for t in v]):
+        return None
+    return tuple(t.value for t in v)
+
+
+_packed_3x3 = _packcache.new_cache("conv3x3_bn_weight")
+
+
+def _packed_3x3_planes(weight):
+    w = weight.detach()
+    state = _packcache.tensor_state(w)
+    hit = _packed_3x3.get(weight, state)
+    if hit is not None:
+        return _lib.keep_for_graph(hit)
+    L = _lib.lib()
+    cout, cin = w.size(0), w.size(1)
+    w32 = w.float().contiguous()
+    packed = torch.empty((L.orp_conv3x3_bn_packed_bytes(cin, cout),), dtype=torch.uint8, device=w.device)
+    with torch.cuda.device(w.device):
+        _lib.check(L.orp_conv3x3_bn_pack_weight(_lib.ptr(w32), cin, cout, _lib.ptr(packed), _lib.stream_of(w32)),
+                   "orp_conv3x3_bn_pack_weight")
+    return _lib.keep_for_graph(_packed_3x3.put(weight, state, packed))
+
+
+def conv3x3_bn_act(x, conv, bn, relu=True, force=False, range_bits=None):
+    if range_bits is None or not conv3x3_bn_act_routed(x, conv, bn, force):
+        return bn_act(conv(x).contiguous(), bn, relu=relu)
+    x = x.detach().contiguous()
+    B, cin, H, W = x.shape
+    cout = conv.weight.size(0)
+    packed = _packed_3x3_planes(conv.weight)
+    scale, shift = _bn_affine(bn)
+    y = torch.empty((B, cout, H, W), dtype=torch.float32, device=x.device)
+    with torch.cuda.device(x.device):
+        rc = _lib.lib().orp_conv3x3_bn_act(_lib.ptr(x), _lib.ptr(packed), _lib.ptr(scale), _lib.ptr(shift), _lib.ptr(range_bits),
+                                           _lib.ptr(y), B, cin, cout, H, W, 1 if relu else 0, _lib.stream_of(x))
+    _lib.check(rc, "orp_conv3x3_bn_act")
     return y
 
 
diff --git a/orientedreppoints_amd/switches.py b/orientedreppoints_amd/switches.py
--- a/orientedreppoints_amd/switches.py
+++ b/orientedreppoints_amd/switches.py
@@ -10,6 +10,7 @@
 TOWER_GN_FUSE = _on('ORP_TOWER_GN_FUSE')
 BN_DOWNSAMPLE_FUSE = _on('ORP_BN_DOWNSAMPLE_FUSE')
 BN_CONV1X1_FUSE = _on('ORP_BN_CONV1X1_FUSE')
+BN_CONV3X3_FUSE = _on('ORP_BN_CONV3X3_FUSE')
 STEM_POOL_FUSE = _on('ORP_STEM_POOL_FUSE')
 FPN_TOPDOWN_FUSE = _on('ORP_FPN_TOPDOWN_FUSE')
 TRAIN_SPLIT = _on('ORP_TRAIN_SPLIT')
```

Measured after the change: 406.5 images/s, median of 6. +9.4%, better.
